# ktncktnc/diffusion-forcing-transformer

Hardware: AMD Instinct MI355X
Metric: denoised latent frames/sec, DFoT RE10K 8f & 200f rollout @1/2/4/8 GPU (higher is better)
Workload: dtype bf16

## Files before the change

diffusion-forcing-transformer_amd/backbone.py:

```python
from __future__ import annotations

import ctypes as C
import math
from typing import Dict, Optional, Sequence, Tuple

import torch
from torch import nn

from . import capi, ops


def _get(cfg, key, default=None):
    if isinstance(cfg, dict):
        return cfg.get(key, default)
    return getattr(cfg, key, default) if not hasattr(cfg, "get") else cfg.get(key, default)


class _Node(nn.Module):
    """Anonymous container so that dotted reference key names map onto a module tree."""


class UViT3DPose(nn.Module):
    def __init__(self, cfg, x_shape: Sequence[int], max_tokens: int, external_cond_dim: int = 0,
                 external_cond_type: str = "action", external_cond_num_classes: Optional[int] = None,
                 use_causal_mask: bool = False, **kwargs):
        super().__init__()
        block_types = list(_get(cfg, "block_types", ["ResBlock", "ResBlock", "TransformerBlock", "TransformerBlock"]))
        if block_types != ["ResBlock", "ResBlock", "TransformerBlock", "TransformerBlock"]:
            raise ValueError(f"unsupported block_types {block_types}")
        if _get(cfg, "pos_emb_type", "rope") != "rope":
            raise ValueError("only pos_emb_type='rope' is supported")
        if not _get(cfg, "use_fourier_noise_embedding", True):
            raise ValueError("only the Fourier noise-level embedding (continuous diffusion) is supported")
        cond = _get(cfg, "conditioning", None)
        cond_dim = _get(cond, "dim", None) if cond is not None else None
        self.cfg = cfg
        self.x_shape = tuple(x_shape)
        self.max_tokens = self.temporal_length = int(max_tokens)
        self.external_cond_dim = int(cond_dim or 180)
        self.use_causal_mask = use_causal_mask
        c = capi.UViTConfig()
        c.channels[:] = list(_get(cfg, "channels"))
        c.emb_channels = int(_get(cfg, "emb_channels"))
        c.num_updown_blocks[:] = list(_get(cfg, "num_updown_blocks"))
        c.num_mid_blocks = int(_get(cfg, "num_mid_blocks"))
        c.num_heads = int(_get(cfg, "num_heads"))
        c.in_channels = int(self.x_shape[0])
        c.resolution = int(self.x_shape[-1])
        c.max_tokens = self.max_tokens
        c.cond_dim = self.external_cond_dim
        c.noise_dim = 256
        c.rope_theta = 10000.0
        c.eps = 1e-6
        if int(_get(cfg, "patch_size", 2)) != 2:
            raise ValueError("only patch_size=2 is supported")
        self._ccfg = c
        self._handle = C.c_void_p()
        capi.check(capi.lib.dfot_uvit_create(C.byref(c), C.byref(self._handle)))
        self._names = []
        self._persistent_buffers = {"noise_level_pos_embedding.timesteps.freqs",
                                    "noise_level_pos_embedding.timesteps.phases"}
        shape = (C.c_int64 * 4)()
        ndim = C.c_int()
        for i in range(capi.lib.dfot_uvit_num_params(self._handle)):
            name = capi.lib.dfot_uvit_param_name(self._handle, i).decode()
            capi.check(capi.lib.dfot_uvit_param_shape(self._handle, i, shape, C.byref(ndim)))
            self._register(name, tuple(shape[k] for k in range(ndim.value)))
            self._names.append(name)
        self._synced: Optional[Tuple] = None
        self._reserved = 0
        self._op_key: Optional[int] = None
        self._cond_key = None
        self._cond_refs = None
        self._cond_gen = None
        self._cond_flag = None
        self.cond_cache_stats = {"builds": 0, "identity_hits": 0, "content_hits": 0}
        self._train_names = None
        self._trainer = None
        self._trainer_sig = None
        self.live_frames = None
        self.fresh_frames = None
        self._fresh_key = None
        self._train_stamp = 0
        self._dropout_generator: Optional[torch.Generator] = None

    def _register(self, name: str, shape: Tuple[int, ...]) -> None:
        *path, leaf = name.split(".")
        node: nn.Module = self
        for part in path:
            if part not in node._modules:
                node.add_module(part, _Node())
            node = node._modules[part]
        t = torch.zeros(shape, dtype=torch.float32)
        if name in self._persistent_buffers:
            node.register_buffer(leaf, t, persistent=True)
        else:
            node.register_parameter(leaf, nn.Parameter(t))

    def _tensors(self) -> Dict[str, torch.Tensor]:
        sd = dict(self.named_parameters())
        sd.update(dict(self.named_buffers()))
        return sd

    def reset_parameters(self, seed: int = 0) -> None:
        g = torch.Generator().manual_seed(seed)
        with torch.no_grad():
            for name, t in self._tensors().items():
                leaf = name.rsplit(".", 1)[-1]
                if leaf == "freqs":
                    t.copy_(2 * math.pi * torch.randn(t.shape, generator=g))
                elif leaf == "phases":
                    t.copy_(2 * math.pi * torch.rand(t.shape, generator=g))
                elif any(s in name for s in (".attn_out.", ".mlp_out.2.", ".out_rest.1.", "project_output")):
                    t.zero_()
                elif leaf == "bias":
                    t.zero_()
                elif t.ndim == 1:
                    t.fill_(1.0)
                else:
                    fan_in = math.prod(t.shape[1:])
                    bound = 1.0 / math.sqrt(fan_in)
                    t.copy_((torch.rand(t.shape, generator=g) * 2 - 1) * bound)

    def _signature(self) -> Tuple:
        return tuple((t.data_ptr(), t._version) for t in self._tensors().values())

    def sync_weights(self, force: bool = False) -> None:
        sig = self._signature()
        if not force and sig == self._synced:
            return
        tensors = self._tensors()
        s = capi.stream_ptr()
        for name in self._names:
            t = tensors[name]
            if not t.is_cuda:
                raise RuntimeError(f"parameter {name} is on {t.device}; move the module to the GPU first")
            src = t.detach().to(torch.float32).contiguous()
            shape = (C.c_int64 * src.ndim)(*src.shape)
            capi.check(capi.lib.dfot_uvit_load_weight(self._handle, name.encode(), capi.ptr(src), shape, src.ndim, s))
        capi.check(capi.lib.dfot_uvit_finalize(self._handle, s))
        self._synced = sig
        self.reserve_generation = getattr(self, "reserve_generation", 0) + 1

    def set_option(self, key: str, value: int) -> None:
        self.reserve_generation = getattr(self, "reserve_generation", 0) + 1
        capi.check(capi.lib.dfot_uvit_set_option(self._handle, key.encode(), int(value)))

    def query(self, key: str) -> float:
        self.sync_weights()
        val = C.c_double()
        capi.check(capi.lib.dfot_uvit_query(self._handle, key.encode(), C.byref(val)))
        return float(val.value)

    def attn_timing(self):
        tot, n = C.c_double(), C.c_int64()
        capi.check(capi.lib.dfot_uvit_attn_timing(self._handle, C.byref(tot), C.byref(n)))
        return tot.value, n.value

    def init_random(self, seed: int = 0, zero_init_scale: float = 0.3) -> None:
        g = torch.Generator().manual_seed(seed)
        with torch.no_grad():
            for name, t in self._tensors().items():
                leaf = name.rsplit(".", 1)[-1]
                if leaf == "freqs":
# ... 10 lines not shown
                    if any(s in name for s in (".attn_out.", ".mlp_out.2.", ".out_rest.1.", "project_output")):
                        v = v * zero_init_scale
                t.copy_(v.to(t.device))

    def reserve(self, batch: int) -> None:
        if batch > self._reserved:
            torch.cuda.synchronize()
            capi.check(capi.lib.dfot_uvit_reserve(self._handle, int(batch)))
            self._reserved = batch
            self.reserve_generation = getattr(self, "reserve_generation", 0) + 1
            self._cond_key = None

    def forward(self, x: torch.Tensor, noise_levels: torch.Tensor, external_cond: Optional[torch.Tensor] = None,
                external_cond_mask: Optional[torch.Tensor] = None) -> torch.Tensor:
        assert external_cond is not None, "External condition (camera pose) is required for U-ViT3DPose model."
        if self._op_key is None:
            self._op_key = ops.register_model(self)
        if torch.is_grad_enabled() and (x.requires_grad or any(p.requires_grad for p in self.parameters())):
            if self._train_names is None:
                self._train_names = [n for n, _ in self.named_parameters()]
            params = [p for _, p in self.named_parameters()]
            return torch.ops.dfot.uvit3d_pose_forward_train(x, noise_levels, external_cond, external_cond_mask, params, self._op_key)
        return torch.ops.dfot.uvit3d_pose_forward(x, noise_levels, external_cond, external_cond_mask, self._op_key)

    def _train_engine(self, params):
        from . import uvit_train
        sig = tuple((t.data_ptr(), t._version) for t in params) + tuple((b.data_ptr(), b._version) for _, b in self.named_buffers())
        if self._trainer is None:
            cfg = dict(channels=list(self._ccfg.channels), emb_channels=int(self._ccfg.emb_channels), patch_size=2,
                       block_types=["ResBlock", "ResBlock", "TransformerBlock", "TransformerBlock"],
                       num_updown_blocks=list(self._ccfg.num_updown_blocks), num_mid_blocks=int(self._ccfg.num_mid_blocks),
                       num_heads=int(self._ccfg.num_heads), in_channels=int(self._ccfg.in_channels), resolution=int(self._ccfg.resolution),
                       max_tokens=self.max_tokens, cond_dim=self.external_cond_dim, noise_dim=int(self._ccfg.noise_dim),
                       eps=float(self._ccfg.eps), rope_theta=float(self._ccfg.rope_theta),
                       block_dropouts=list(_get(self.cfg, "block_dropouts", [0.0] * 4) or [0.0] * 4))
            sd = {n: t for n, t in zip(self._train_names, params)}
            sd.update(dict(self.named_buffers()))
            ordered = {n: sd[n] for n in self._names}
            self._trainer = uvit_train.UViT3DPoseTrainer(ordered, cfg)
            self._trainer_sig = sig
        elif sig != self._trainer_sig:
            with torch.no_grad():
                for n, t in zip(self._train_names, params):
                    self._trainer.p[n].copy_(t)
                for n, b in self.named_buffers():
                    self._trainer.p[n].copy_(b)
            self._trainer.sync()
            self._trainer_sig = sig
        return self._trainer

    def _train_forward_impl(self, x, noise_levels, external_cond, external_cond_mask, params):
        assert x.shape[1] == self.temporal_length, (
            f"Temporal length of U-ViT is set to {self.temporal_length}, but input has temporal length {x.shape[1]}.")
        dev = params[0].device
        if dev.type != "cuda":
            raise RuntimeError(f"the backbone's parameters are on {dev}; move the module to the GPU first (there is no CPU path)")
        capi.require_device(dev, x=x, noise_levels=noise_levels, external_cond=external_cond, external_cond_mask=external_cond_mask)
        eng = self._train_engine(params)
        drop = external_cond_mask
        pdrop = float(_get(self.cfg, "external_cond_dropout", 0.0) or 0.0)
        if drop is None and self.training and pdrop > 0:
            drop = torch.rand(x.shape[0], device=dev) < pdrop
        eng.dropout_generator = self._dropout_generator if self.training else None
        self._train_stamp += 1
        with torch.no_grad():
            return eng.forward(x, noise_levels, external_cond, drop).to(x.dtype)

    def _train_backward_impl(self, grad_out, params, stamp=None, want_dx=False):
        eng = self._trainer
        if eng is None:
            raise RuntimeError("backward without a training forward")
        if stamp is not None and stamp != self._train_stamp:
            raise RuntimeError(
                f"UViT3DPose: backward of training forward #{stamp}, but forward #{self._train_stamp} has run since and overwritten the "
                "saved activations (one engine per module). Run backward after each forward (accumulate gradients as forward/backward "
                "pairs); two forwards of one module inside one loss are not supported.")
        with torch.no_grad():
            grads = eng.backward(grad_out, input_grad=want_dx)
        out = [grads[n].to(p.dtype).reshape(p.shape) if n in grads else torch.zeros_like(p) for n, p in zip(self._train_names, params)]
        if want_dx:
            out.append(eng.dx_in.to(grad_out.dtype))
        return out

    def _cond_content_equal(self, cond: torch.Tensor, mask: Optional[torch.Tensor]) -> bool:
        if self._cond_key is None or self._cond_refs is None:
            return False
        kept, kept_mask = self._cond_refs
        _, version, shape, synced, mask_key = self._cond_key
        if synced != self._synced or self._cond_gen != self.reserve_generation:
            return False
        if kept._version != version or (kept_mask is not None and kept_mask._version != mask_key[1]):
            return False
        for t in (cond, kept):
            if t.dtype != torch.float32 or not t.is_contiguous():
                return False
        if cond.device != kept.device or tuple(cond.shape) != shape:
            return False
        if (mask is None) != (kept_mask is None):
            return False
        if mask is not None and (mask.dtype != kept_mask.dtype or mask.shape != kept_mask.shape or mask.device != kept_mask.device
                                 or not mask.is_contiguous() or not kept_mask.is_contiguous()):
            return False
        if torch.cuda.is_current_stream_capturing():
            return False
        if self._cond_flag is None or self._cond_flag.device != cond.device:
            self._cond_flag = torch.zeros(1, dtype=torch.int32, device=cond.device)
        flag = self._cond_flag
        flag.zero_()
        s = capi.stream_ptr()
        capi.check(capi.lib.dfot_op_equal_bits(capi.ptr(kept), capi.ptr(cond), cond.numel() * cond.element_size(), capi.ptr(flag), s))
        if mask is not None:
            capi.check(capi.lib.dfot_op_equal_bits(capi.ptr(kept_mask), capi.ptr(mask), mask.numel() * mask.element_size(), capi.ptr(flag), s))
        return int(flag.item()) == 0

    def _forward_impl(self, x: torch.Tensor, noise_levels: torch.Tensor, external_cond: Optional[torch.Tensor] = None,
                      external_cond_mask: Optional[torch.Tensor] = None) -> torch.Tensor:
        assert x.shape[1] == self.temporal_length, (
            f"Temporal length of U-ViT is set to {self.temporal_length}, but input has temporal length {x.shape[1]}.")
        assert external_cond is not None, "External condition (camera pose) is required for U-ViT3DPose model."
        b = x.shape[0]
        if tuple(x.shape[2:]) != self.x_shape:
            raise ValueError(f"x has frame shape {tuple(x.shape[2:])}, expected {self.x_shape}")
        if tuple(external_cond.shape) != (b, self.temporal_length, self.external_cond_dim, *self.x_shape[1:]):
            raise ValueError(f"external_cond has shape {tuple(external_cond.shape)}")
        if external_cond_mask is not None:
            assert external_cond_mask.ndim == 1, "embedding mask should be of shape (B,)"
        if tuple(noise_levels.shape) != (b, self.temporal_length):
            raise ValueError(f"noise_levels has shape {tuple(noise_levels.shape)}, expected {(b, self.temporal_length)}")
        dev = next(self.parameters()).device
        if dev.type != "cuda":
            raise RuntimeError(f"the backbone's parameters are on {dev}; move the module to the GPU first (there is no CPU path)")
        capi.require_device(dev, x=x, noise_levels=noise_levels, external_cond=external_cond, external_cond_mask=external_cond_mask)
        self.sync_weights()
        self.reserve(b)
        xf = x.detach().to(torch.float32).contiguous()
        kf = noise_levels.detach().to(torch.float32).contiguous()
        key = (external_cond.data_ptr(), external_cond._version, tuple(external_cond.shape), self._synced,
               None if external_cond_mask is None else (external_cond_mask.data_ptr(), external_cond_mask._version))
        if key == self._cond_key:
            self.cond_cache_stats["identity_hits"] += 1
        else:
            if self._cond_content_equal(external_cond, external_cond_mask):
                self.cond_cache_stats["content_hits"] += 1
            else:
                cf = external_cond.detach().to(torch.float32).contiguous()
                mf = None if external_cond_mask is None else external_cond_mask.to(torch.uint8).contiguous()
                capi.check(capi.lib.dfot_uvit_set_conditions(self._handle, capi.ptr(cf, torch.float32, "external_cond"),
                                                             capi.ptr(mf, torch.uint8, "external_cond_mask"), b, capi.stream_ptr()))
                self.cond_cache_stats["builds"] += 1
            self._cond_key = key
            self._cond_refs = (external_cond, external_cond_mask)
            self._cond_gen = self.reserve_generation
        out = torch.empty_like(xf)
        live = self.live_frames
        if live is not None:
            if tuple(live.shape) != (b, self.temporal_length) or live.dtype != torch.uint8 or not live.is_contiguous():
                raise ValueError(f"live_frames must be a contiguous uint8 tensor of shape {(b, self.temporal_length)}")
            capi.require_device(dev, live_frames=live)
        fresh = self.fresh_frames
        if fresh is not None:
            if tuple(fresh.shape) != (b, self.temporal_length) or fresh.dtype != torch.uint8 or not fresh.is_contiguous():
                raise ValueError(f"fresh_frames must be a contiguous uint8 tensor of shape {(b, self.temporal_length)}")
            capi.require_device(dev, fresh_frames=fresh)
            if key != self._fresh_key:
                fresh = None
        capi.check(capi.lib.dfot_uvit_forward_cached_masks(self._handle, capi.ptr(xf, torch.float32, "x"),
                                                           capi.ptr(kf, torch.float32, "noise_levels"), capi.ptr(out), b,
                                                           capi.ptr(live, torch.uint8, "live_frames"),
                                                           capi.ptr(fresh, torch.uint8, "fresh_frames"), capi.stream_ptr()))
        self._fresh_key = key
        return out.to(x.dtype)

    def read_tap(self, name: str, channels: int, level: int, batch: int) -> torch.Tensor:
        r = self.x_shape[-1] // 2 // (2 ** level)
        out = torch.empty(batch * self.temporal_length, channels, r, r, device="cuda", dtype=torch.float32)
        capi.check(capi.lib.dfot_uvit_read_tap(self._handle, name.encode(), capi.ptr(out), out.numel(), capi.stream_ptr()))
        return out

    def __del__(self):
        try:
            if getattr(self, "_handle", None) and self._handle.value:
                capi.lib.dfot_uvit_destroy(self._handle)
                self._handle = C.c_void_p()
        except Exception:
            pass
```

diffusion-forcing-transformer_amd/capi.py:

```python
from __future__ import annotations

import ctypes as C
import os

_HERE = os.path.dirname(os.path.abspath(__file__))
LIB_PATH = os.environ.get("DFOT_LIB", os.path.join(_HERE, "libdfot_hip.so"))

OK, ERR_ARG, ERR_SHAPE, ERR_HIP, ERR_STATE, ERR_NAME = range(6)


class DfotError(RuntimeError):
    def __init__(self, code: int, message: str):
        super().__init__(f"libdfot_hip error {code}: {message}")
        self.code = code


class UViTConfig(C.Structure):
    _fields_ = [
        ("channels", C.c_int32 * 4), ("emb_channels", C.c_int32), ("num_updown_blocks", C.c_int32 * 3),
        ("num_mid_blocks", C.c_int32), ("num_heads", C.c_int32), ("in_channels", C.c_int32),
        ("resolution", C.c_int32), ("max_tokens", C.c_int32), ("cond_dim", C.c_int32), ("noise_dim", C.c_int32),
        ("rope_theta", C.c_float), ("eps", C.c_float),
    ]


class UViT3DConfig(C.Structure):
    _fields_ = UViTConfig._fields_ + [("cond_dropout", C.c_int32)]


class DiTConfig(C.Structure):
    _fields_ = [
        ("hidden_size", C.c_int32), ("depth", C.c_int32), ("num_heads", C.c_int32), ("patch_size", C.c_int32),
        ("in_channels", C.c_int32), ("height", C.c_int32), ("width", C.c_int32), ("max_tokens", C.c_int32),
        ("mlp_hidden", C.c_int32), ("noise_dim", C.c_int32), ("timesteps", C.c_int32),
        ("rope_theta", C.c_float), ("eps", C.c_float),
        ("variant", C.c_int32), ("embed_col_dim", C.c_int32), ("num_col_heads", C.c_int32), ("num_row_heads", C.c_int32),
        ("temporal_mlp_hidden", C.c_int32), ("use_bias", C.c_int32),
        ("cond_type", C.c_int32), ("cond_dim", C.c_int32), ("num_classes", C.c_int32), ("cond_dropout", C.c_int32),
        ("use_temporal_rope", C.c_int32),
    ]


class DiTConfigF(DiTConfig):
    _fields_ = [("fourier_noise", C.c_int32)]


COND_NONE, COND_ACTION, COND_LABEL = 0, 1, 2
ATTN_MAP_OFF, ATTN_MAP_FRAME, ATTN_MAP_FULL = -1, 0, 1


_P, _I, _L, _F = C.c_void_p, C.c_int, C.c_int64, C.c_float
_I32 = C.c_int32


class GemmDesc(C.Structure):
    _fields_ = [
        ("amode", _I32), ("epi", _I32), ("variant", _I32),
        ("A", _P), ("lda", _L), ("W", _P), ("ldw", _L),
        ("M", _I32), ("N", _I32), ("K", _I32), ("H", _I32), ("Wd", _I32), ("Cin", _I32),
        ("live", _P), ("bias", _P), ("bias_rows", _I32),
        ("out_f32", _P), ("out_bf16", _P), ("ldo", _L),
        ("resid", _P), ("resid_bf", _P),
        ("gate", _P), ("gate_index", _P), ("ldg", _L), ("gate_rows", _I32),
        ("act", _I32), ("pre_act", _P), ("raw", _P), ("ldraw", _L), ("tr_rows", _I32),
        ("gn_part", _P), ("gn_rows_per_bt", _I32), ("gn_cpg", _I32),
        ("out2", _P), ("ldo2", _L), ("split", _I32),
        ("q", _P), ("k", _P), ("v", _P),
        ("qw", _P), ("kw", _P), ("rope_cs", _P),
        ("heads", _I32), ("d", _I32), ("ntok", _I32), ("qscale", _F), ("dstride", _I32), ("eps", _F),
        ("ksplit", _I32), ("slice_stride", _L),
    ]


SIGNATURES = {
    "dfot_last_error": (C.c_char_p, []),
    "dfot_version": (_I, []),
    "dfot_uvit_create": (_I, [C.POINTER(UViTConfig), C.POINTER(_P)]),
    "dfot_uvit_destroy": (_I, [_P]),
    "dfot_uvit_num_params": (_I, [_P]),
    "dfot_uvit_param_name": (C.c_char_p, [_P, _I]),
    "dfot_uvit_param_shape": (_I, [_P, _I, C.POINTER(_L), C.POINTER(_I)]),
    "dfot_uvit_load_weight": (_I, [_P, C.c_char_p, _P, C.POINTER(_L), _I, _P]),
    "dfot_uvit_finalize": (_I, [_P, _P]),
    "dfot_uvit_reserve": (_I, [_P, _I]),
    "dfot_uvit_workspace_bytes": (C.c_size_t, [_P]),
    "dfot_uvit_set_option": (_I, [_P, C.c_char_p, _I]),
    "dfot_uvit_query": (_I, [_P, C.c_char_p, C.POINTER(C.c_double)]),
    "dfot_uvit_attn_timing": (_I, [_P, C.POINTER(C.c_double), C.POINTER(_L)]),
    "dfot_uvit_forward": (_I, [_P, _P, _P, _P, _P, _P, _I, _P]),
    "dfot_uvit_set_conditions": (_I, [_P, _P, _P, _I, _P]),
    "dfot_uvit_forward_cached": (_I, [_P, _P, _P, _P, _I, _P]),
    "dfot_uvit_forward_cached_live": (_I, [_P, _P, _P, _P, _I, _P, _P]),
    "dfot_uvit_forward_cached_masks": (_I, [_P, _P, _P, _P, _I, _P, _P, _P]),
    "dfot_uvit_read_tap": (_I, [_P, C.c_char_p, _P, C.c_size_t, _P]),
    "dfot_uvit3d_create": (_I, [C.POINTER(UViT3DConfig), C.POINTER(_P)]),
    "dfot_uvit3d_config_bytes": (_L, []),
    "dfot_uvit3d_forward": (_I, [_P, _P, _P, _P, _P, _P, _I, _P]),
    "dfot_uvit3d_forward_live": (_I, [_P, _P, _P, _P, _P, _P, _I, _P, _P]),
    "dfot_op_gn_film_silu": (_I, [_P, _P, _P, _P, _P, _P, _P, _P, _I, _I, _I, _I, _P]),
    "dfot_op_rms_film": (_I, [_P, _P, _P, _P, _P, _P, _L, _I, _I, _I, _F, _P]),
    "dfot_dit_create": (_I, [C.POINTER(DiTConfig), C.POINTER(_P)]),
    "dfot_dit_create_f": (_I, [C.POINTER(DiTConfigF), C.POINTER(_P)]),
    "dfot_dit_destroy": (_I, [_P]),
    "dfot_dit_num_params": (_I, [_P]),
    "dfot_dit_param_name": (C.c_char_p, [_P, _I]),
    "dfot_dit_param_shape": (_I, [_P, _I, C.POINTER(_L), C.POINTER(_I)]),
    "dfot_dit_load_weight": (_I, [_P, C.c_char_p, _P, C.POINTER(_L), _I, _P]),
    "dfot_dit_finalize": (_I, [_P, _P]),
    "dfot_dit_reserve": (_I, [_P, _I]),
    "dfot_dit_workspace_bytes": (C.c_size_t, [_P]),
    "dfot_dit_set_option": (_I, [_P, C.c_char_p, _I]),
    "dfot_dit_attn_timing": (_I, [_P, C.POINTER(C.c_double), C.POINTER(_L)]),
    "dfot_dit_forward": (_I, [_P, _P, _P, _P, _I, _I, _P]),
    "dfot_dit_forward_cond": (_I, [_P, _P, _P, _P, _P, _P, _P, _I, _I, _P]),
    "dfot_dit_forward_f": (_I, [_P, _P, _P, _P, _P, _P, _P, _I, _I, _P]),
    "dfot_dit_read_tap": (_I, [_P, C.c_char_p, _P, C.c_size_t, _P]),
    "dfot_dit_capture_attention": (_I, [_P, C.POINTER(_I32), _I, _I, C.c_size_t]),
    "dfot_dit_attention_map_shape": (_I, [_P, _I, C.POINTER(_L), C.POINTER(_I)]),
    "dfot_dit_read_attention_map": (_I, [_P, _I, _P, C.c_size_t, _P]),
    "dfot_dit_train_create": (_I, [C.POINTER(DiTConfig), C.POINTER(_P)]),
    "dfot_dit_train_create_f": (_I, [C.POINTER(DiTConfigF), C.POINTER(_P)]),
    "dfot_facmat_train_create": (_I, [C.POINTER(DiTConfigF), C.POINTER(_P)]),
    "dfot_facdit_train_create": (_I, [C.POINTER(DiTConfigF), C.POINTER(_P)]),
    "dfot_dit_train_destroy": (_I, [_P]),
    "dfot_dit_train_num_params": (_I, [_P]),
    "dfot_dit_train_param_name": (C.c_char_p, [_P, _I]),
    "dfot_dit_train_param_shape": (_I, [_P, _I, C.POINTER(_L), C.POINTER(_I)]),
    "dfot_dit_train_param_offset": (_L, [_P, _I]),
    "dfot_dit_train_total_numel": (_L, [_P]),
    "dfot_dit_train_workspace_bytes": (C.c_size_t, [_P]),
    "dfot_dit_train_attach": (_I, [_P, _P, _P]),
    "dfot_dit_train_reserve": (_I, [_P, _I]),
    "dfot_dit_train_sync_weights": (_I, [_P, _P]),
    "dfot_dit_train_forward": (_I, [_P, _P, _P, _P, _I, _I, _P]),
    "dfot_dit_train_forward_cond": (_I, [_P, _P, _P, _P, _P, _P, _P, _I, _I, _P]),
    "dfot_dit_train_load_buffer": (_I, [_P, C.c_char_p, _P, _L, _P]),
    "dfot_dit_train_forward_f": (_I, [_P, _P, _P, _P, _P, _P, _P, _I, _I, _P]),
    "dfot_dit_train_input_grad": (_I, [_P, _P, _P]),
    "dfot_dit_train_backward": (_I, [_P, _P, _P]),
    "dfot_vloss_grad": (_I, [_P] * 7 + [_I, _I, _L, _I, _P]),
    "dfot_sumsq": (_I, [_P, _L, _P, _P]),
    "dfot_adamw_step": (_I, [_P, _P, _P, _P, _L, _F, _F, _F, _F, _F, _I, _P, _F, _P, _F, _P]),
    "dfot_ray_encode": (_I, [_P, _P, _I, _I, _I, _P]),
    "dfot_ray_encode_normalized": (_I, [_P, _P, _I, _I, _I, _P]),
    "dfot_hg_prepare": (_I, [_P, _P, _P, _P, _P, _I, _I, _I, _L, _P]),
    "dfot_ddim_compose": (_I, [_P] * 11 + [_I, _I, _I, _L, _P]),
    "dfot_ddim_compose_tokw": (_I, [_P] * 11 + [_I, _I, _I, _L, _P]),
    "dfot_ddim_noise": (_I, [_P] * 5 + [_I, _I, _I, _L, _I, _P]),
    "dfot_vpred_loss": (_I, [_P] * 9 + [_I, _I, _L, _P]),
    "dfot_vpred_loss_scratch_floats": (_L, [_I, _I, _L]),
    "dfot_vspace_loss": (_I, [_P] * 9 + [_I, _I, _L, _P]),
    "dfot_op_gemm": (_I, [_P, _I, _P, _P, _P, _I, _I, _I, _I, _P]),
    "dfot_op_conv3x3": (_I, [_P, _P, _P, _P, _I, _I, _I, _I, _I, _I, _P]),
    "dfot_op_gemm_ex": (_I, [C.POINTER(GemmDesc), _P]),
    "dfot_op_gemm_desc_bytes": (_L, []),
    "dfot_op_attention": (_I, [_P, _P, _P, _P, _I, _I, _I, _I, _I, _I, _P]),
    "dfot_op_attention_padded": (_I, [_P, _P, _P, _P, _I, _I, _I, _I, _I, _P]),
    "dfot_op_attention_seq64": (_I, [_P, _P, _P, _P, _I, _I, _I, _I, _P]),
    "dfot_op_attention_temporal": (_I, [_P, _P, _P, _P, _I, _I, _I, _I, _I, _I, _P]),
    "dfot_op_attention_temporal_bwd": (_I, [_P, _P, _P, _P, _I, _P, _P, _P, _I, _I, _I, _I, _I, _P]),
    "dfot_op_matrix_attention_rope": (_I, [_P, _P, _P, _I, _I, _I, _I, _I, _I, _F, _P]),
    "dfot_op_matrix_attention_rope_bwd": (_I, [_P, _P, _P, _P, _I, _I, _I, _I, _I, _I, _F, _P]),
    "dfot_op_attention_map_workspace_bytes": (C.c_size_t, [_I, _I, _I, _I, _I]),
    "dfot_op_attention_map": (_I, [_P, _P, _P, _P, C.c_size_t, _I, _I, _I, _I, _I, _I, _P]),
    "dfot_op_attention_temporal_map": (_I, [_P, _P, _P, _P, C.c_size_t, _I, _I, _I, _I, _I, _P]),
    "dfot_op_matrix_attention_map": (_I, [_P, _P, _P, _I, _I, _I, _I, _I, _I, _F, _P]),
    "dfot_op_matrix_attention": (_I, [_P, _P, _I, _I, _I, _I, _I, _I, _F, _P]),
    "dfot_op_facmat_contract": (_I, [_P, _P, _P, _I, _I, _I, _I, _P]),
    "dfot_op_facmat_expand": (_I, [_P, _P, _P, _I, _I, _I, _I, _P]),
    "dfot_op_attention_bwd": (_I, [_P, _P, _P, _P, _P, _I, _P, _P, _P, _I, _I, _I, _I, _P]),
    "dfot_op_conv3x3_bwd": (_I, [_P, _P, _P, _P, _P, _P, _I, _I, _I, _I, _I, _P]),
    "dfot_op_conv3x3_bwd2": (_I, [_P, _P, _P, _P, _P, _P, _P, _I, _I, _I, _I, _I, _P]),
    "dfot_op_gn_silu_bwd": (_I, [_P, _P, _P, _P, _P, _F, _P, _P, _P, _P, _I, _I, _I, _P]),
    "dfot_op_rms_film_bwd": (_I, [_P, _P, _P, _P, _F, _P, _P, _P, _L, _I, _I, _P]),
    "dfot_op_rms_film_bwd_res": (_I, [_P, _P, _P, _P, _F, _P, _P, _P, _P, _P, _L, _I, _P]),
    "dfot_op_qknorm_rope_bwd": (_I, [_P, _I, _P, _P, _P, _P, _P, _P, _F, _P, _I, _P, _P, _L, _I, _I, _I, _P]),
    "dfot_op_wgrad_nt": (_I, [_P, _I, _P, _I, _P, _I, _I, _L, _I, _P]),
    "dfot_op_gemm_bf16": (_I, [_P, _I, _P, _P, _P, _I, _I, _I, _I, _P]),
    "dfot_op_gemm_f32": (_I, [_P, _I, _P, _P, _P, _P, _I, _I, _I, _I, _P]),
    "dfot_op_transpose_bf16": (_I, [_P, _P, _I, _I, _P]),
    "dfot_op_colsum_bf16": (_I, [_P, _I, _P, _L, _I, _P]),
    "dfot_op_rms_film_fwd": (_I, [_P, _P, _P, _F, _P, _L, _I, _P]),
    "dfot_op_qknorm_rope_fwd": (_I, [_P, _I, _P, _P, _P, _F, _F, _P, _P, _P, _L, _I, _I, _I, _P]),
# ... 116 lines not shown
```

diffusion-forcing-transformer_amd/csrc/kernels.h:

```cpp
#pragma once
#include "common.h"

namespace dfot {

int launch_noise_emb(const float* k, const float* freqs, const float* phases, const float* w1, const float* b1,
                     const float* w2, const float* b2, float* hidden, float* out, int bt, int ndim, int e, hipStream_t s);
int launch_uvit3d_emb(const float* k, const float* freqs, const float* phases, const float* w1, const float* b1, const float* w2,
                      const float* b2, const float* cond, const uint8_t* cond_mask, const float* a_w1, const float* a_b1,
                      const float* a_w2, const float* a_b2, float* out, int bt, int ndim, int cdim, int e, int tokens, hipStream_t s);
int launch_embed_input(const float* x, const float* w, const float* b, float* out, int bt, int res, int cin, int c0,
                       hipStream_t s);
int launch_cond_repack(const float* cond, bf16* a, int bt, int res, int cdim, int kpad, hipStream_t s);
int launch_emb_pyramid(const bf16* emb0, bf16* emb1, bf16* emb2, bf16* emb3, int bt, int r0, int e, hipStream_t s);
int launch_project_output(const float* x0, const float* w, const float* b, float* out, int bt, int res, int c0, int cout,
                          hipStream_t s, const uint8_t* live = nullptr);
int launch_gn_partial_f32(const float* x, float* partial, int bt, int pixels, int c, hipStream_t s);
int launch_gn_partial_bf16(const bf16* x, float* partial, int bt, int pixels, int c, hipStream_t s);
int launch_gn_finalize(const float* partial, float* stats, int bt, int nblk, int pixels, int c, float eps, hipStream_t s);
int gn_partial_blocks(int pixels);
int launch_gn_apply_silu(const float* x, const float* stats, const float* gamma, const float* beta, bf16* out, int bt,
                         int pixels, int c, hipStream_t s, const uint8_t* live = nullptr);
struct FilmChunk {
  const bf16* w;
  const float* b;
  long out_off;
  int rows;
};
int launch_film_vec(const FilmChunk* table, int chunks, const float* nemb, float* sv, int bt, int e, hipStream_t s);
int launch_gn_film_silu(const bf16* h, const float* stats, const float* gamma, const float* beta, const bf16* fcache,
                        const float* sv, const uint8_t* cond_mask, bf16* out, int bt, int pixels, int c, int tokens,
                        hipStream_t s, const uint8_t* live = nullptr);
struct RmsPending {
  void* x;
  const float* bias;
  const float* s0;
  const float* s1;
  const float* s2;
};
int launch_rms_film(const float* x, const float* w, const bf16* fcache, const float* sv, const uint8_t* cond_mask, bf16* out,
                    long m, int c, int rows_per_bt, int tokens, float eps, hipStream_t s, const RmsPending* pend = nullptr);
int launch_rms_film_bf16(const bf16* x, const float* w, const bf16* fcache, const float* sv, const uint8_t* cond_mask, bf16* out,
                         long m, int c, int rows_per_bt, int tokens, float eps, hipStream_t s, const RmsPending* pend = nullptr);

int launch_pool2_bf16(const float* x, bf16* out, int bt, int h, int w, int c, hipStream_t s);
int launch_pool2_bf16_bf16in(const bf16* x, bf16* out, int bt, int h, int w, int c, hipStream_t s);
int launch_sub_bf16_bf16in(const bf16* a, const float* b, bf16* out, long n, hipStream_t s, const uint8_t* live = nullptr, long frame_elems = 0);
int launch_upsample_add_bf16(const float* t, const bf16* skip, bf16* out, int bt, int h, int w, int c, hipStream_t s, const uint8_t* live = nullptr);
int launch_gn_apply_silu_bf16in(const bf16* x, const float* stats, const float* gamma, const float* beta, bf16* out, int bt, int pixels, int c,
                                hipStream_t s, const uint8_t* live = nullptr);
int launch_embed_input_bf16(const float* x, const float* w, const float* b, bf16* out, int bt, int res, int cin, int c0, hipStream_t s);
int launch_project_output_bf16(const bf16* x0, const float* w, const float* b, float* out, int bt, int res, int c0, int cout, hipStream_t s,
                               const uint8_t* live = nullptr);
int launch_sub_bf16(const float* a, const float* b, bf16* out, long n, hipStream_t s, const uint8_t* live = nullptr, long frame_elems = 0);
int launch_upsample_add(const float* t, const float* skip, float* out, int bt, int h, int w, int c, hipStream_t s, const uint8_t* live = nullptr);
int launch_ray_encode(const float* poses, float* out, int b, int t, int res, int normalized, hipStream_t s);
int launch_hg_prepare(const float* x, const float* noise, const float* qa, const float* qb, float* x_in, int batch,
                      int nfe, int tokens, long f, hipStream_t s);
int launch_ddim_compose(const float* x, const float* x_in, const float* v, const float* sa, const float* s1,
                        const float* an, const float* cn, const float* keep, const float* weight, const uint8_t* gen,
                        float* x_next, int batch, int nfe, int tokens, long f, bool weight_per_token, hipStream_t s);
int launch_ddim_noise(const float* noise, const float* sigma, const float* weight, const uint8_t* gen, float* x_next, int batch, int nfe,
                      int tokens, long f, bool weight_per_token, hipStream_t s);
int vloss_chunks(long f);
int launch_vloss(const float* x, const float* noise, const float* v, const float* a, const float* sg, const float* w,
                 float* x_pred, float* partial, float* loss, int batch, int tokens, long f, bool vspace, hipStream_t s);
int launch_wgrad_nt(const bf16* a, long lda, const bf16* b, long ldb, float* out, int m, int n, long rows, int slices, hipStream_t s, int img_h = 0,
                    int img_w = 0, int sdy = 0, int sdx = 0, int all_taps = 0);
struct WgradPlan {
  int form, slices;
};
WgradPlan wgrad_plan(int m, int n, long rows, long max_slices);
int launch_wgrad_conv_taps(const bf16* dy, const bf16* x, float* out, int co, int ci, long pix, int slices, int img_h, int img_w, hipStream_t s);
int wgrad_conv_tiles(int co, int ci, int* target);
int launch_wgrad_nt_plan(const bf16* a, long lda, const bf16* b, long ldb, float* out, int m, int n, long rows, WgradPlan plan, hipStream_t s);
int launch_vloss_grad(const float* x, const float* noise, const float* v, const float* a, const float* sg, const float* coef, float* dv,
                      int batch, int tokens, long f, bool vspace, hipStream_t s);
int launch_sumsq(const float* x, long n, float* out, hipStream_t s);
int launch_adamw(float* p, const float* g, float* m, float* v, long n, float lr, float b1, float b2, float eps, float wd, int step,
                 const float* sumsq, float max_norm, float* ema, float ema_decay, hipStream_t s);
int launch_f32_to_bf16(const float* src, bf16* dst, long n, hipStream_t s);
int launch_bf16_to_f32(const bf16* src, float* dst, long n, hipStream_t s);
int launch_equal_bits(const void* a, const void* b, long bytes, int* differs, hipStream_t s);
int launch_pack_rows(const float* src, bf16* dst, const int* map, int rows, int k, int kpad, long ldd, int col0,
                     hipStream_t s);
int launch_pack_conv3(const float* src, bf16* dst, int co, int ci, hipStream_t s);
int launch_gather_f32(const float* src, float* dst, const int* map, int n, hipStream_t s);
int launch_nhwc_to_nchw(const float* src, float* dst, int bt, int p, int c, hipStream_t s);
int launch_bf16_nhwc_to_nchw(const bf16* src, float* dst, int bt, int p, int c, hipStream_t s);

struct AttnScratch {
  float* p = nullptr;
  size_t bytes = 0;
};
int launch_attention(const bf16* q, const bf16* k, const bf16* v, bf16* o, long ldo, int batch, int heads, int n, int d,
                     int variant, hipStream_t stream, AttnScratch* scratch = nullptr);
int launch_attention_v3(const bf16* q, const bf16* k, const bf16* v, bf16* o, long ldo, int batch, int heads, int n, bool nomax,
                        hipStream_t stream, AttnScratch* scratch = nullptr);
bool attention_v5_applies(int n, int d, float score_bound);
int launch_attention_v5(const bf16* q, const bf16* k, const bf16* v, bf16* o, long ldo, int batch, int heads, int n, hipStream_t stream,
                        AttnScratch* scratch = nullptr, float* lse = nullptr);
bool attention_ks_applies(int batch, int heads, int n, int d);
size_t attention_ks_scratch_bytes(int batch, int heads, int n, int d);
int launch_attention_ks(const bf16* q, const bf16* k, const bf16* v, bf16* o, long ldo, int batch, int heads, int n, hipStream_t stream,
                        AttnScratch* scratch = nullptr);
int attention_dstride(int d);
int launch_attention_padded(const bf16* q, const bf16* k, const bf16* v, bf16* o, long ldo, int batch, int heads, int n, int d,
                            hipStream_t stream, float* lse = nullptr);
int launch_attention_seq64(const bf16* q, const bf16* k, const bf16* v, bf16* o, long ldo, int nseq, int heads, int d, hipStream_t stream);
int launch_attention_temporal(const bf16* q, const bf16* k, const bf16* v, bf16* o, long ldo, int batch, int tokens, int patches, int heads,
                              int d, hipStream_t s);
int launch_attention_temporal_bwd(const bf16* q, const bf16* k, const bf16* v, const bf16* d_o, long ldo, bf16* dq, bf16* dk, bf16* dv,
                                  int batch, int tokens, int patches, int heads, int d, hipStream_t s);
int launch_matrix_attn_rope(const bf16* z, bf16* o, const float* rope_cs, int batch, int L, int E, int h, int cc, int rr, float scale,
                            hipStream_t s);
int launch_matrix_attn_rope_bwd(const bf16* z, const bf16* d_o, const float* rope_cs, bf16* dz, int batch, int L, int E, int h, int cc, int rr,
                                float scale, hipStream_t s);
int launch_facmat_contract(const bf16* m, const bf16* u, bf16* w, int frames, int P, int h, int E, hipStream_t s);
int launch_facmat_expand(const bf16* o, const bf16* u, bf16* sp, int frames, int P, int h, int E, hipStream_t s);
size_t attention_map_part_floats(int batch, int heads, int n, int tokens);
int launch_attention_map(const bf16* q, const bf16* k, float* out, float* part, bool full, int batch, int heads, int n, int tokens, int d,
                         hipStream_t s);
size_t attention_temporal_map_part_floats(int batch, int heads, int tokens, int patches);
int launch_attention_temporal_map(const bf16* q, const bf16* k, float* out, float* part, int batch, int tokens, int patches, int heads, int d,
                                  hipStream_t s);
int launch_matrix_attn_map(const bf16* z, const float* rope_cs, float* out, int batch, int L, int E, int h, int cc, int rr, float scale,
// ... 17 lines not shown
```

diffusion-forcing-transformer_amd/csrc/kernels.hip:

```cpp
#include "kernels.h"
#include "dfot_hip.h"

namespace dfot {

typedef __attribute__((ext_vector_type(4))) float float4v;
typedef __attribute__((ext_vector_type(2))) float float2v;

__device__ __forceinline__ float wave_sum(float v) {
#pragma unroll
  for (int o = 32; o > 0; o >>= 1) v += __shfl_xor(v, o);
  return v;
}

template <bool FOURIER>
__global__ __launch_bounds__(256) void noise_mlp_kernel(const float* __restrict__ in, const float* __restrict__ freqs,
                                                        const float* __restrict__ phases, const float* __restrict__ w,
                                                        const float* __restrict__ b, float* __restrict__ out, int kdim,
                                                        int e) {
  const int lane = threadIdx.x & 63, wave = threadIdx.x >> 6;
  const int row = blockIdx.x * 4 + wave;
  const int bt = blockIdx.y;
  if (row >= e) return;
  float acc = 0.f;
  for (int i = lane; i < kdim; i += 64) {
// ... 638 lines not shown
    const float* ne = nemb + (long)bt * e;
    float acc = 0.f;
#pragma unroll
    for (int k = 0; k < 2; ++k) {
      const int i = lane * 8 + k * 512;
      if (i < e) {
        const float4v a = *reinterpret_cast<const float4v*>(ne + i);
        const float4v b = *reinterpret_cast<const float4v*>(ne + i + 4);
        acc += wv[k][0] * a[0] + wv[k][1] * a[1] + wv[k][2] * a[2] + wv[k][3] * a[3] + wv[k][4] * b[0] + wv[k][5] * b[1] +
               wv[k][6] * b[2] + wv[k][7] * b[3];
      }
    }
    acc = wave_sum(acc);
    if (lane == 0) sv[ck.out_off + (long)bt * ck.rows + r] = acc + bias;
  }
}
template <int EQ>
__global__ __launch_bounds__(256, 2) void film_vec_lds_kernel(const FilmChunk* __restrict__ table, const float* __restrict__ nemb,
                                                           float* __restrict__ sv, int nbt) {
  constexpr int E = EQ * 256;
  __shared__ float4v ne[16][E / 4];
  const FilmChunk ck = table[blockIdx.x >> 1];
  const int lane = threadIdx.x & 63, wave = threadIdx.x >> 6;
  for (int bt0 = 0; bt0 < nbt; bt0 += 16) {
    __syncthreads();
    for (int i = threadIdx.x; i < 16 * (E / 4); i += 256) {
      const int f = i / (E / 4);
      float4v v = {0.f, 0.f, 0.f, 0.f};
      if (bt0 + f < nbt) v = reinterpret_cast<const float4v*>(nemb + (long)(bt0 + f) * E)[i % (E / 4)];
      ne[f][i % (E / 4)] = v;
    }
    __syncthreads();
#pragma unroll 1
    for (int pass = 0; pass < 4; ++pass) {
      const int r0 = (blockIdx.x & 1) * 32 + pass * 8 + wave * 2;
      float wv[2][EQ][4];
#pragma unroll
      for (int r = 0; r < 2; ++r)
#pragma unroll
        for (int k = 0; k < EQ; ++k) {
          const bf16x4 t = *reinterpret_cast<const bf16x4*>(ck.w + (long)(r0 + r) * E + k * 256 + lane * 4);
#pragma unroll
          for (int j = 0; j < 4; ++j) wv[r][k][j] = bf2f(t[j]);
        }
      float acc[32];
#pragma unroll
      for (int f = 0; f < 16; ++f) {
        float4v x[EQ];
#pragma unroll
        for (int k = 0; k < EQ; ++k) x[k] = ne[f][k * 64 + lane];
#pragma unroll
        for (int r = 0; r < 2; ++r) {
          float a = 0.f;
#pragma unroll
          for (int k = 0; k < EQ; ++k) a += wv[r][k][0] * x[k][0] + wv[r][k][1] * x[k][1] + wv[r][k][2] * x[k][2] + wv[r][k][3] * x[k][3];
          acc[r * 16 + f] = a;
        }
        if ((f & 3) == 3) __builtin_amdgcn_sched_barrier(0);
      }
      halve_exchange<16, 32>(acc, lane);
      halve_exchange<8, 16>(acc, lane);
      halve_exchange<4, 8>(acc, lane);
      halve_exchange<2, 4>(acc, lane);
      halve_exchange<1, 2>(acc, lane);
      const float v = acc[0] + __shfl_xor(acc[0], 1);
      const int r = r0 + (lane >> 5), f = bt0 + ((lane >> 1) & 15);
      if (f < nbt && (lane & 1) == 0) sv[ck.out_off + (long)f * ck.rows + r] = v + ck.b[r];
    }
  }
}
int launch_film_vec(const FilmChunk* table, int chunks, const float* nemb, float* sv, int bt, int e, hipStream_t s) {
  DFOT_REQUIRE(e % 8 == 0 && e <= 1024, DFOT_ERR_SHAPE, "film_vec: emb dim %d must be a multiple of 8 and <= 1024", e);
  if (e == 1024 || e == 512) {
    if (e == 1024) hipLaunchKernelGGL(film_vec_lds_kernel<4>, dim3(chunks * 2), dim3(256), 0, s, table, nemb, sv, bt);
    else hipLaunchKernelGGL(film_vec_lds_kernel<2>, dim3(chunks * 2), dim3(256), 0, s, table, nemb, sv, bt);
    DFOT_CHECK_HIP(hipGetLastError());
    return DFOT_OK;
  }
  hipLaunchKernelGGL(film_vec_kernel, dim3(chunks * 16), dim3(256), 0, s, table, nemb, sv, e, bt);
  DFOT_CHECK_HIP(hipGetLastError());
  return DFOT_OK;
}

template <bool POSE>
__global__ void gn_film_silu_kernel(const bf16* __restrict__ h, const float* __restrict__ stats,
                                    const float* __restrict__ gamma, const float* __restrict__ beta,
                                    const bf16* __restrict__ fcache, const float* __restrict__ sv,
                                    const uint8_t* __restrict__ cond_mask, bf16* __restrict__ out, long total8, int pixels,
                                    int c, int tokens, const uint8_t* __restrict__ live) {
  const long idx = (long)blockIdx.x * blockDim.x + threadIdx.x;
  if (idx >= total8) return;
  const unsigned iu = (unsigned)idx, cq = (unsigned)(c / 8);
  const int c8 = (int)(iu % cq);
  const long pix = iu / cq;
  const int bt = (int)((unsigned)pix / (unsigned)pixels);
  if (live && !live[bt]) return;
  const int cpg = c / 32;
  const int c0 = c8 * 8;
  const int col = (c0 >> 5) * 64 + (c0 & 31);
  const bf16x8 hv = *reinterpret_cast<const bf16x8*>(h + pix * c + c0);
  const float* svp = sv + (long)bt * 2 * c + col;
  float sc[8], sh[8];
#pragma unroll
  for (int j = 0; j < 8; ++j) {
    sc[j] = svp[j];
    sh[j] = svp[32 + j];
  }
  if constexpr (POSE) {
    const bool use_pose = !(cond_mask && cond_mask[(unsigned)bt / (unsigned)tokens]);
    if (use_pose) {
      const bf16x8 fs = *reinterpret_cast<const bf16x8*>(fcache + pix * 2 * c + col);
      const bf16x8 fh = *reinterpret_cast<const bf16x8*>(fcache + pix * 2 * c + col + 32);
#pragma unroll
      for (int j = 0; j < 8; ++j) {
        sc[j] += bf2f(fs[j]);
        sh[j] += bf2f(fh[j]);
      }
    }
  }
  bf16x8 o;
#pragma unroll
  for (int j = 0; j < 8; ++j) {
    const int ch = c0 + j;
    const int g = ch / cpg;
    const float mean = stats[(bt * 32 + g) * 2], rs = stats[(bt * 32 + g) * 2 + 1];
    const float y = ((bf2f(hv[j]) - mean) * rs * gamma[ch] + beta[ch]) * (1.f + sc[j]) + sh[j];
    o[j] = f2bf(silu_f(y));
  }
  *reinterpret_cast<bf16x8*>(out + pix * c + c0) = o;
}
template <int C, bool POSE>
__global__ __launch_bounds__(256) void gn_film_silu_rows_kernel(const bf16* __restrict__ h, const float* __restrict__ stats,
                                                                const float* __restrict__ gamma, const float* __restrict__ beta,
                                                                const bf16* __restrict__ fcache, const float* __restrict__ sv,
                                                                const uint8_t* __restrict__ cond_mask, bf16* __restrict__ out, int pixels,
                                                                int tokens, const uint8_t* __restrict__ live) {
  constexpr int TPP = C / 8, PPI = 256 / TPP;
  const int wg_per_bt = pixels / (PPI * GN_ROWS_IT);
  const int bt = blockIdx.x / wg_per_bt;
  if (live && !live[bt]) return;
  const int c0 = (threadIdx.x % TPP) * 8;
  const int col = (c0 >> 5) * 64 + (c0 & 31);
  GnRowConsts<C> k;
  k.load(stats, gamma, beta, bt, c0);
  const float* svp = sv + (long)bt * 2 * C + col;
  float svs[8], svh[8];
  {
    const float4v s0 = *reinterpret_cast<const float4v*>(svp), s1 = *reinterpret_cast<const float4v*>(svp + 4);
    const float4v h0 = *reinterpret_cast<const float4v*>(svp + 32), h1 = *reinterpret_cast<const float4v*>(svp + 36);
#pragma unroll
    for (int j = 0; j < 8; ++j) {
      svs[j] = j < 4 ? s0[j] : s1[j - 4];
      svh[j] = j < 4 ? h0[j] : h1[j - 4];
    }
  }
  bool use_pose = false;
  if constexpr (POSE) use_pose = !(cond_mask && cond_mask[(unsigned)bt / (unsigned)tokens]);
  long pix = (long)bt * pixels + (long)(blockIdx.x % wg_per_bt) * (PPI * GN_ROWS_IT) + threadIdx.x / TPP;
  if (POSE && use_pose) {
#pragma unroll 4
    for (int it = 0; it < GN_ROWS_IT; ++it, pix += PPI) {
      const bf16x8 hv = *reinterpret_cast<const bf16x8*>(h + pix * C + c0);
      const bf16x8 fs = *reinterpret_cast<const bf16x8*>(fcache + pix * 2 * C + col);
      const bf16x8 fh = *reinterpret_cast<const bf16x8*>(fcache + pix * 2 * C + col + 32);
      bf16x8 o;
#pragma unroll
      for (int j = 0; j < 8; ++j) {
        const float sc = svs[j] + bf2f(fs[j]), sh = svh[j] + bf2f(fh[j]);
        o[j] = f2bf(silu_f(k.norm(bf2f(hv[j]), j) * (1.f + sc) + sh));
      }
      *reinterpret_cast<bf16x8*>(out + pix * C + c0) = o;
    }
  } else {
#pragma unroll 4
    for (int it = 0; it < GN_ROWS_IT; ++it, pix += PPI) {
      const bf16x8 hv = *reinterpret_cast<const bf16x8*>(h + pix * C + c0);
      bf16x8 o;
#pragma unroll
      for (int j = 0; j < 8; ++j) o[j] = f2bf(silu_f(k.norm(bf2f(hv[j]), j) * (1.f + svs[j]) + svh[j]));
      *reinterpret_cast<bf16x8*>(out + pix * C + c0) = o;
    }
  }
}

template <bool POSE>
static int launch_gn_film_silu_t(const bf16* h, const float* stats, const float* gamma, const float* beta, const bf16* fcache,
                                 const float* sv, const uint8_t* cond_mask, bf16* out, int bt, int pixels, int c, int tokens,
                                 hipStream_t s, const uint8_t* live) {
  if ((c == 128 || c == 256) && pixels % ((256 / (c / 8)) * GN_ROWS_IT) == 0) {
    const int grid = bt * (pixels / ((256 / (c / 8)) * GN_ROWS_IT));
    if (c == 128)
      hipLaunchKernelGGL((gn_film_silu_rows_kernel<128, POSE>), dim3(grid), dim3(256), 0, s, h, stats, gamma, beta, fcache, sv, cond_mask, out, pixels, tokens, live);
    else
      hipLaunchKernelGGL((gn_film_silu_rows_kernel<256, POSE>), dim3(grid), dim3(256), 0, s, h, stats, gamma, beta, fcache, sv, cond_mask, out, pixels, tokens, live);
    DFOT_CHECK_HIP(hipGetLastError());
    return DFOT_OK;
  }
  const long total8 = (long)bt * pixels * (c / 8);
  DFOT_REQUIRE(total8 < (1L << 31), DFOT_ERR_SHAPE, "groupnorm apply: %ld work items exceed the 32-bit index range", total8);
  hipLaunchKernelGGL(gn_film_silu_kernel<POSE>, dim3(cdiv(total8, 256)), dim3(256), 0, s, h, stats, gamma, beta, fcache, sv,
                     cond_mask, out, total8, pixels, c, tokens, live);
  DFOT_CHECK_HIP(hipGetLastError());
  return DFOT_OK;
}
int launch_gn_film_silu(const bf16* h, const float* stats, const float* gamma, const float* beta, const bf16* fcache,
                        const float* sv, const uint8_t* cond_mask, bf16* out, int bt, int pixels, int c, int tokens,
                        hipStream_t s, const uint8_t* live) {
  return fcache ? launch_gn_film_silu_t<true>(h, stats, gamma, beta, fcache, sv, cond_mask, out, bt, pixels, c, tokens, s, live)
                : launch_gn_film_silu_t<false>(h, stats, gamma, beta, nullptr, sv, nullptr, out, bt, pixels, c, tokens, s, live);
}

template <int MAXCH, bool PEND, typename TS, bool POSE>
__global__ __launch_bounds__(256) void rms_film_kernel(const TS* x, const float* __restrict__ w,
                                                       const bf16* __restrict__ fcache, const float* __restrict__ sv,
                                                       const uint8_t* __restrict__ cond_mask, bf16* __restrict__ out,
                                                       long m, int c, int rows_per_bt, int tokens, float eps, TS* xw,
                                                       const float* __restrict__ pbias, const float* __restrict__ p0,
                                                       const float* __restrict__ p1, const float* __restrict__ p2) {
  const long row = (long)blockIdx.x * 4 + (threadIdx.x >> 6);
  if (row >= m) return;
  const int lane = threadIdx.x & 63;
  const int nch = c / 8;
  const TS* src = x + row * c;
  float v[MAXCH][8];
  float ss = 0.f;
#pragma unroll
  for (int k = 0; k < MAXCH; ++k) {
    const int ch = lane + 64 * k;
    if (ch < nch) {
      stream_ld8(src + ch * 8, v[k]);
      if constexpr (PEND) {
        const long o = row * c + ch * 8;
#pragma unroll
        for (int hf = 0; hf < 2; ++hf) {
          float4v add = *reinterpret_cast<const float4v*>(pbias + ch * 8 + 4 * hf) + *reinterpret_cast<const float4v*>(p0 + o + 4 * hf) +
                        *reinterpret_cast<const float4v*>(p1 + o + 4 * hf);
          if (p2) add += *reinterpret_cast<const float4v*>(p2 + o + 4 * hf);
#pragma unroll
          for (int j = 0; j < 4; ++j) v[k][4 * hf + j] += add[j];
        }
        stream_st8(xw + o, v[k]);
        if constexpr (sizeof(TS) == 2) {
#pragma unroll
          for (int j = 0; j < 8; ++j) v[k][j] = bf2f(f2bf(v[k][j]));
        }
      }
#pragma unroll
      for (int j = 0; j < 8; ++j) ss += v[k][j] * v[k][j];
    }
  }
  ss = wave_sum(ss);
  const float rs = rsqrtf(ss / (float)c + eps);
  const int bt = (int)(row / rows_per_bt);
  bool use_pose = false;
  if constexpr (POSE) use_pose = !(cond_mask && cond_mask[(unsigned)bt / (unsigned)tokens]);
#pragma unroll
  for (int k = 0; k < MAXCH; ++k) {
    const int ch = lane + 64 * k;
    if (ch < nch) {
      const int c0 = ch * 8;
      const int col = (c0 >> 5) * 64 + (c0 & 31);
      const float* svp = sv + (long)bt * 2 * c + col;
      float sc[8], sh[8];
#pragma unroll
      for (int j = 0; j < 8; ++j) {
        sc[j] = svp[j];
        sh[j] = svp[32 + j];
      }
      if (POSE && use_pose) {
        const bf16x8 fs = *reinterpret_cast<const bf16x8*>(fcache + row * 2 * c + col);
        const bf16x8 fh = *reinterpret_cast<const bf16x8*>(fcache + row * 2 * c + col + 32);
#pragma unroll
        for (int j = 0; j < 8; ++j) {
          sc[j] += bf2f(fs[j]);
          sh[j] += bf2f(fh[j]);
        }
      }
      bf16x8 o;
#pragma unroll
      for (int j = 0; j < 8; ++j) o[j] = f2bf(v[k][j] * rs * w[c0 + j] * (1.f + sc[j]) + sh[j]);
      *reinterpret_cast<bf16x8*>(out + row * c + c0) = o;
    }
  }
}
template <typename TS, bool POSE>
static int launch_rms_film_p(const TS* x, const float* w, const bf16* fcache, const float* sv, const uint8_t* cond_mask, bf16* out,
                             long m, int c, int rows_per_bt, int tokens, float eps, hipStream_t s, const RmsPending* pend) {
  DFOT_REQUIRE(c % 8 == 0 && c <= 8 * 64 * 3, DFOT_ERR_SHAPE, "rms_film: channels %d unsupported", c);
#define RMS_CALL(MC, P)                                                                                                             \
  hipLaunchKernelGGL((rms_film_kernel<MC, P, TS, POSE>), dim3(cdiv(m, 4)), dim3(256), 0, s, x, w, fcache, sv, cond_mask, out, m, c, rows_per_bt, \
                     tokens, eps, P ? (TS*)pend->x : nullptr, P ? pend->bias : nullptr, P ? pend->s0 : nullptr, P ? pend->s1 : nullptr, P ? pend->s2 : nullptr)
  if (pend) {
    DFOT_REQUIRE(pend->x && pend->bias && pend->s0 && pend->s1, DFOT_ERR_ARG, "rms_film: pending sum needs a target, a bias and two slices");
    if (c <= 8 * 64 * 2) RMS_CALL(2, true); else RMS_CALL(3, true);
  } else {
    if (c <= 8 * 64 * 2) RMS_CALL(2, false); else RMS_CALL(3, false);
  }
#undef RMS_CALL
  DFOT_CHECK_HIP(hipGetLastError());
  return DFOT_OK;
}
template <typename TS>
static int launch_rms_film_t(const TS* x, const float* w, const bf16* fcache, const float* sv, const uint8_t* cond_mask, bf16* out,
                             long m, int c, int rows_per_bt, int tokens, float eps, hipStream_t s, const RmsPending* pend) {
  return fcache ? launch_rms_film_p<TS, true>(x, w, fcache, sv, cond_mask, out, m, c, rows_per_bt, tokens, eps, s, pend)
                : launch_rms_film_p<TS, false>(x, w, nullptr, sv, nullptr, out, m, c, rows_per_bt, tokens, eps, s, pend);
}
int launch_rms_film(const float* x, const float* w, const bf16* fcache, const float* sv, const uint8_t* cond_mask, bf16* out,
                    long m, int c, int rows_per_bt, int tokens, float eps, hipStream_t s, const RmsPending* pend) {
  return launch_rms_film_t<float>(x, w, fcache, sv, cond_mask, out, m, c, rows_per_bt, tokens, eps, s, pend);
}
int launch_rms_film_bf16(const bf16* x, const float* w, const bf16* fcache, const float* sv, const uint8_t* cond_mask, bf16* out,
                         long m, int c, int rows_per_bt, int tokens, float eps, hipStream_t s, const RmsPending* pend) {
  return launch_rms_film_t<bf16>(x, w, fcache, sv, cond_mask, out, m, c, rows_per_bt, tokens, eps, s, pend);
}

template <typename TIN>
__global__ void pool2_bf16_kernel(const TIN* __restrict__ x, bf16* __restrict__ out, long total4, int h, int w, int c) {
  const long idx = (long)blockIdx.x * blockDim.x + threadIdx.x;
  if (idx >= total4) return;
  const unsigned iu = (unsigned)idx, cq = (unsigned)(c / 4), w2 = (unsigned)(w / 2), h2 = (unsigned)(h / 2);
  const int c4 = (int)(iu % cq);
  const unsigned pix = iu / cq;
  const int ox = (int)(pix % w2), oy = (int)((pix / w2) % h2);
  const long bt = pix / (w2 * h2);
  const TIN* base = x + ((bt * h + 2 * oy) * w + 2 * ox) * (long)c + c4 * 4;
  const float4v a = stream_ld4(base);
  const float4v b = stream_ld4(base + c);
  const float4v cc = stream_ld4(base + (long)w * c);
  const float4v dd = stream_ld4(base + (long)w * c + c);
  bf16x4 o;
#pragma unroll
  for (int j = 0; j < 4; ++j) o[j] = f2bf((a[j] + b[j] + cc[j] + dd[j]) * 0.25f);
  *reinterpret_cast<bf16x4*>(out + pix * c + c4 * 4) = o;
}
int launch_pool2_bf16(const float* x, bf16* out, int bt, int h, int w, int c, hipStream_t s) {
  const long total4 = (long)bt * (h / 2) * (w / 2) * (c / 4);
  DFOT_REQUIRE(total4 < (1L << 31), DFOT_ERR_SHAPE, "pool2: %ld work items exceed the 32-bit index range", total4);
  hipLaunchKernelGGL(pool2_bf16_kernel<float>, dim3(cdiv(total4, 256)), dim3(256), 0, s, x, out, total4, h, w, c);
  DFOT_CHECK_HIP(hipGetLastError());
  return DFOT_OK;
}
int launch_pool2_bf16_bf16in(const bf16* x, bf16* out, int bt, int h, int w, int c, hipStream_t s) {
  const long total4 = (long)bt * (h / 2) * (w / 2) * (c / 4);
  DFOT_REQUIRE(total4 < (1L << 31), DFOT_ERR_SHAPE, "pool2: %ld work items exceed the 32-bit index range", total4);
  hipLaunchKernelGGL(pool2_bf16_kernel<bf16>, dim3(cdiv(total4, 256)), dim3(256), 0, s, x, out, total4, h, w, c);
  DFOT_CHECK_HIP(hipGetLastError());
  return DFOT_OK;
}

template <typename TIN, typename TB = TIN>
__global__ void sub_bf16_kernel(const TIN* __restrict__ a, const TB* __restrict__ b, bf16* __restrict__ out, long n4,
                                const uint8_t* __restrict__ live, long frame4) {
  const long idx = (long)blockIdx.x * blockDim.x + threadIdx.x;
  if (idx >= n4) return;
  if (live && !live[idx / frame4]) return;
  const float4v x = stream_ld4(a + idx * 4);
  const float4v y = stream_ld4(b + idx * 4);
  bf16x4 o;
#pragma unroll
  for (int j = 0; j < 4; ++j) o[j] = f2bf(x[j] - y[j]);
  *reinterpret_cast<bf16x4*>(out + idx * 4) = o;
}
int launch_sub_bf16(const float* a, const float* b, bf16* out, long n, hipStream_t s, const uint8_t* live, long frame_elems) {
  DFOT_REQUIRE(n % 4 == 0 && (!live || (frame_elems > 0 && frame_elems % 4 == 0)), DFOT_ERR_SHAPE, "sub: length %ld must be a multiple of 4", n);
  hipLaunchKernelGGL((sub_bf16_kernel<float, float>), dim3(cdiv(n / 4, 256)), dim3(256), 0, s, a, b, out, n / 4, live, live ? frame_elems / 4 : 1L);
  DFOT_CHECK_HIP(hipGetLastError());
  return DFOT_OK;
}
int launch_sub_bf16_bf16in(const bf16* a, const float* b, bf16* out, long n, hipStream_t s, const uint8_t* live, long frame_elems) {
  DFOT_REQUIRE(n % 4 == 0 && (!live || (frame_elems > 0 && frame_elems % 4 == 0)), DFOT_ERR_SHAPE, "sub: length %ld must be a multiple of 4", n);
  hipLaunchKernelGGL((sub_bf16_kernel<bf16, float>), dim3(cdiv(n / 4, 256)), dim3(256), 0, s, a, b, out, n / 4, live, live ? frame_elems / 4 : 1L);
  DFOT_CHECK_HIP(hipGetLastError());
  return DFOT_OK;
}

template <typename TS>
__global__ void upsample_add_kernel(const float* __restrict__ t, const TS* __restrict__ skip, TS* __restrict__ out,
                                    long total4, int h, int w, int c, const uint8_t* __restrict__ live) {
  const long idx = (long)blockIdx.x * blockDim.x + threadIdx.x;
  if (idx >= total4) return;
  const unsigned iu = (unsigned)idx, cq = (unsigned)(c / 4), w2 = (unsigned)(2 * w), h2 = (unsigned)(2 * h);
  const int c4 = (int)(iu % cq);
  const unsigned pix = iu / cq;
  const int x = (int)(pix % w2), y = (int)((pix / w2) % h2);
  const long bt = pix / (w2 * h2);
  if (live && !live[bt]) return;
  const float4v a = *reinterpret_cast<const float4v*>(t + ((bt * h + y / 2) * w + x / 2) * (long)c + c4 * 4);
  const float4v b = stream_ld4(skip + pix * c + c4 * 4);
  stream_st4(out + pix * c + c4 * 4, a + b);
}
int launch_upsample_add(const float* t, const float* skip, float* out, int bt, int h, int w, int c, hipStream_t s, const uint8_t* live) {
  const long total4 = (long)bt * 4 * h * w * (c / 4);
  DFOT_REQUIRE(total4 < (1L << 31), DFOT_ERR_SHAPE, "upsample_add: %ld work items exceed the 32-bit index range", total4);
  hipLaunchKernelGGL(upsample_add_kernel<float>, dim3(cdiv(total4, 256)), dim3(256), 0, s, t, skip, out, total4, h, w, c, live);
  DFOT_CHECK_HIP(hipGetLastError());
  return DFOT_OK;
// ... 495 lines not shown
```

diffusion-forcing-transformer_amd/csrc/uvit.hip:

```cpp
#include <algorithm>
#include <cmath>
#include <cstdarg>
#include <cstdlib>
#include <cstring>
#include <functional>
#include <map>
#include <string>
#include <vector>

#include "dfot_hip.h"
#include "gemm.h"
#include "kernels.h"

namespace dfot {

static thread_local char g_err[1024] = "";
void set_error(const char* fmt, ...) {
  va_list ap;
  va_start(ap, fmt);
  vsnprintf(g_err, sizeof(g_err), fmt, ap);
  va_end(ap);
}
const char* get_error() { return g_err; }

int tuning_flag(const char* name, int dflt) {
  std::string key = std::string("DFOT_") + name;
  const char* v = getenv(key.c_str());
  return v ? atoi(v) : dflt;
}

struct ResW {
  int c = 0;
  bf16* fcache = nullptr;
  long sv_off = 0;
  bf16 *w_film = nullptr, *w1 = nullptr, *w2 = nullptr;
  float *b_film_raw = nullptr, *b_film = nullptr, *g1 = nullptr, *be1 = nullptr, *bias1 = nullptr, *g2 = nullptr,
        *be2 = nullptr, *bias2 = nullptr;
};
struct TrW {
  int c = 0;
  bf16* fcache = nullptr;
  long sv_off = 0;
  bf16 *w_film = nullptr, *w_fused = nullptr, *w_out = nullptr;
  float *b_film_raw = nullptr, *b_film = nullptr, *nw = nullptr, *b_fused = nullptr, *qw = nullptr, *kw = nullptr,
        *b_attn = nullptr, *b_mlp = nullptr, *b_out = nullptr;
  float score_bound = INFINITY;
};
struct ConvW {
  int cin = 0, cout = 0;
  bf16* w = nullptr;
  float* b = nullptr;
};

struct Param {
  std::string name;
  std::vector<int64_t> shape;
  std::function<int(const float*, hipStream_t)> load;
  bool loaded = false;
};

}

using namespace dfot;

struct dfot_uvit_s {
  dfot_uvit_config cfg{};
  int T = 0, E = 0, heads = 0, r[4] = {0, 0, 0, 0}, ch[4] = {0, 0, 0, 0};
  int kpose = 0;
  bool posefree = false;
  int act_dim = 0;
  bool act_dropout = false;
  float *ac_w1 = nullptr, *ac_b1 = nullptr, *ac_w2 = nullptr, *ac_b2 = nullptr;
  std::vector<Param> params;
  std::map<std::string, int> index;
  std::vector<void*> owned;

  float *ne_freqs = nullptr, *ne_phases = nullptr, *ne_w1 = nullptr, *ne_b1 = nullptr, *ne_w2 = nullptr, *ne_b2 = nullptr;
  bf16* pose_w = nullptr;
  float* pose_b = nullptr;
  float *ein_w = nullptr, *ein_b = nullptr, *pout_w = nullptr, *pout_b = nullptr;
  std::vector<ResW> down_res[2], up_res[2];
  std::vector<TrW> down_tr, mid_tr, up_tr;
  ConvW down_conv[3], up_conv[3];
  int* film_map[4] = {nullptr, nullptr, nullptr, nullptr};
  float* rope_cs[4] = {nullptr, nullptr, nullptr, nullptr};
  bf16* zeros = nullptr;
  bool finalized = false;

  int max_batch = 0;
  size_t ws_bytes = 0;
  std::vector<void*> ws_owned;
  float *nemb = nullptr, *nhid = nullptr, *X[4] = {nullptr, nullptr, nullptr, nullptr}, *HSA[3] = {nullptr, nullptr, nullptr}, *tmp = nullptr,
        *gn_partial = nullptr, *gn_partial2 = nullptr, *gn_stats = nullptr, *sv = nullptr;
  int gn1_nblk = 0;
  FilmChunk* film_table = nullptr;
  int film_chunks = 0;
  uint8_t* cond_mask = nullptr;
  bool have_mask = false;
  int cond_batch = 0;
  int64_t cond_builds = 0;
  bf16 *acond = nullptr, *emb[4] = {nullptr, nullptr, nullptr, nullptr}, *s1 = nullptr, *hbf = nullptr,
       *cat = nullptr, *q = nullptr, *k = nullptr, *v = nullptr;
  AttnScratch attn_scratch;
  const float* pend_part = nullptr;
  float* out_part = nullptr;
  size_t out_part_elems = 0;
  const float* pend_bias = nullptr;
  int pend_lvl = 0, pend_c = 0, pend_slices = 2;
  long pend_m = 0;
  int last_batch = 0;
  const float* xin[4] = {nullptr, nullptr, nullptr, nullptr};
  bf16* XB[4] = {nullptr, nullptr, nullptr, nullptr};
  bool xin_bf[4] = {false, false, false, false};
  int gemm_variant = GEMM_AUTO;
  int attn_variant = 2;
  bool attn_force_safe = false;
  bool time_attn = false;
  std::vector<hipEvent_t> ev_start, ev_stop;
  size_t ev_used = 0;
};

namespace dfot {

template <typename T>
static int dev_alloc(dfot_uvit_s* h, T** out, size_t count, bool workspace = false) {
  void* p = nullptr;
  const size_t bytes = count * sizeof(T);
  DFOT_CHECK_HIP(hipMalloc(&p, bytes ? bytes : 16));
  (workspace ? h->ws_owned : h->owned).push_back(p);
  if (workspace) h->ws_bytes += bytes;
  *out = reinterpret_cast<T*>(p);
  return DFOT_OK;
}

static int copy_f32(float* dst, const float* src, size_t n, hipStream_t s) {
  DFOT_CHECK_HIP(hipMemcpyAsync(dst, src, n * sizeof(float), hipMemcpyDeviceToDevice, s));
  return DFOT_OK;
}

static void add_param(dfot_uvit_s* h, const std::string& name, std::vector<int64_t> shape,
                      std::function<int(const float*, hipStream_t)> load) {
  h->index[name] = (int)h->params.size();
  h->params.push_back(Param{name, std::move(shape), std::move(load), false});
}

static int add_f32(dfot_uvit_s* h, const std::string& name, std::vector<int64_t> shape, float** dst) {
  size_t n = 1;
  for (auto d : shape) n *= (size_t)d;
  int rc = dev_alloc(h, dst, n);
  if (rc) return rc;
  float* d = *dst;
  add_param(h, name, shape, [d, n](const float* src, hipStream_t s) { return copy_f32(d, src, n, s); });
  return DFOT_OK;
}

static int add_res_block(dfot_uvit_s* h, const std::string& pre, int c, ResW* w) {
  const int e = h->E;
  w->c = c;
  int rc = 0;
  if ((rc = dev_alloc(h, &w->w_film, (size_t)2 * c * e))) return rc;
  if ((rc = dev_alloc(h, &w->b_film_raw, (size_t)2 * c))) return rc;
  if ((rc = dev_alloc(h, &w->b_film, (size_t)2 * c))) return rc;
  if ((rc = dev_alloc(h, &w->w1, (size_t)c * 9 * c))) return rc;
  if ((rc = dev_alloc(h, &w->w2, (size_t)c * 9 * c))) return rc;
  const int lvl = c == h->ch[0] ? 0 : 1;
  int* map = h->film_map[lvl];
  bf16* wf = w->w_film;
  add_param(h, pre + ".emb_layer.weight", {2 * c, e, 1, 1}, [=](const float* src, hipStream_t s) {
    return launch_pack_rows(src, wf, map, 2 * c, e, e, e, 0, s);
  });
  float *braw = w->b_film_raw, *bre = w->b_film;
  add_param(h, pre + ".emb_layer.bias", {2 * c}, [=](const float* src, hipStream_t s) {
    int r2 = copy_f32(braw, src, 2 * c, s);
    return r2 ? r2 : launch_gather_f32(braw, bre, map, 2 * c, s);
  });
  if ((rc = add_f32(h, pre + ".in_layers.0.weight", {c}, &w->g1))) return rc;
  if ((rc = add_f32(h, pre + ".in_layers.0.bias", {c}, &w->be1))) return rc;
  bf16* w1 = w->w1;
  add_param(h, pre + ".in_layers.2.weight", {c, c, 3, 3}, [=](const float* src, hipStream_t s) { return launch_pack_conv3(src, w1, c, c, s); });
  if ((rc = add_f32(h, pre + ".in_layers.2.bias", {c}, &w->bias1))) return rc;
  if ((rc = add_f32(h, pre + ".out_norm.weight", {c}, &w->g2))) return rc;
  if ((rc = add_f32(h, pre + ".out_norm.bias", {c}, &w->be2))) return rc;
// ... 122 lines not shown
  }
  auto add_mid = [&]() -> int {
    h->mid_tr.resize(c.num_mid_blocks);
    for (int i = 0; i < c.num_mid_blocks; ++i)
      if ((rc = add_tr_block(h, "mid_blocks." + std::to_string(i), 3, &h->mid_tr[i]))) return rc;
    return DFOT_OK;
  };
  if (!h->posefree && (rc = add_mid())) return rc;
  for (int j = 0; j < 3; ++j) {
    const int l = 2 - j;
    const int n = c.num_updown_blocks[l];
    const std::string pre = "up_blocks." + std::to_string(j) + ".";
    if ((rc = add_conv(h, pre + "0.conv", h->ch[l + 1], h->ch[l], &h->up_conv[l]))) return rc;
    if (l < 2) {
      h->up_res[l].resize(n);
      for (int i = 0; i < n; ++i)
        if ((rc = add_res_block(h, pre + std::to_string(i + 1), h->ch[l], &h->up_res[l][i]))) return rc;
    } else {
      h->up_tr.resize(n);
      for (int i = 0; i < n; ++i)
        if ((rc = add_tr_block(h, pre + std::to_string(i + 1), l, &h->up_tr[i]))) return rc;
    }
  }
  if (h->posefree && (rc = add_mid())) return rc;
  return DFOT_OK;
}

static int build_rope(dfot_uvit_s* h, int lvl) {
  const int d = h->ch[lvl] / h->heads, half = d / 2;
  const int q = half / 3, rem = half % 3;
  int parts[3] = {q, q, q};
  if (rem == 1) parts[0] = q + 1;
  if (rem == 2) parts[1] = parts[2] = q + 1;
  const int rr = h->r[lvl], n = h->T * rr * rr;
  std::vector<float> cs((size_t)n * half * 2);
  for (int tok = 0; tok < n; ++tok) {
    const int pos[3] = {tok / (rr * rr), (tok / rr) % rr, tok % rr};
    int pair = 0;
    for (int ax = 0; ax < 3; ++ax) {
      const int dim = 2 * parts[ax];
      for (int j = 0; j < parts[ax]; ++j, ++pair) {
        const float inv = 1.0f / powf(h->cfg.rope_theta, (float)(2 * j) / (float)dim);
        const float ang = (float)pos[ax] * inv;
        cs[((size_t)tok * half + pair) * 2 + 0] = cosf(ang);
        cs[((size_t)tok * half + pair) * 2 + 1] = sinf(ang);
      }
    }
  }
  int rc = dev_alloc(h, &h->rope_cs[lvl], cs.size());
  if (rc) return rc;
  DFOT_CHECK_HIP(hipMemcpy(h->rope_cs[lvl], cs.data(), cs.size() * sizeof(float), hipMemcpyHostToDevice));
  return DFOT_OK;
}

__global__ void add_vec_kernel(const float* a, const float* b, float* o, int n) {
  const int i = blockIdx.x * blockDim.x + threadIdx.x;
  if (i < n) o[i] = a[i] + b[i];
}

static int run_res_block(dfot_uvit_s* h, const ResW& w, int lvl, int bt, hipStream_t s, const uint8_t* live = nullptr) {
  const int c = w.c, rr = h->r[lvl], pix = rr * rr;
  const int m = bt * pix;
  const int slots = pix / 64;
  bf16* xb = h->XB[lvl];
  int rc = 0;
  if (!h->xin_bf[lvl]) {
    if ((rc = launch_f32_to_bf16(h->xin[lvl], xb, (long)m * c, s))) return rc;
    h->xin_bf[lvl] = true;
  }
  if (h->gn1_nblk == 0) {
    if ((rc = launch_gn_partial_bf16(xb, h->gn_partial, bt, pix, c, s))) return rc;
    h->gn1_nblk = gn_partial_blocks(pix);
  }
  if ((rc = launch_gn_finalize(h->gn_partial, h->gn_stats, bt, h->gn1_nblk, pix, c, h->cfg.eps, s))) return rc;
  h->gn1_nblk = 0;
  if ((rc = launch_gn_apply_silu_bf16in(xb, h->gn_stats, w.g1, w.be1, h->s1, bt, pix, c, s, live))) return rc;
  GemmArgs g;
  g.A = h->s1; g.W = w.w1; g.M = m; g.N = c; g.K = 9 * c; g.H = rr; g.Wd = rr; g.Cin = c; g.zeros = h->zeros;
  g.bias = w.bias1; g.out_bf16 = h->hbf; g.ldo = c; g.live = live;
  g.gn_part = h->gn_partial2; g.gn_rows_per_bt = pix; g.gn_cpg = c / 32;
  if ((rc = launch_gemm(A_CONV3, E_BF16, h->gemm_variant, g, s))) return rc;
  if ((rc = launch_gn_finalize(h->gn_partial2, h->gn_stats, bt, slots, pix, c, h->cfg.eps, s))) return rc;
  if ((rc = launch_gn_film_silu(h->hbf, h->gn_stats, w.g2, w.be2, w.fcache, h->sv + w.sv_off,
                                h->have_mask ? h->cond_mask : nullptr, h->s1, bt, pix, c, h->T, s, live)))
    return rc;
  GemmArgs o;
  o.A = h->s1; o.W = w.w2; o.M = m; o.N = c; o.K = 9 * c; o.H = rr; o.Wd = rr; o.Cin = c; o.zeros = h->zeros;
  o.bias = w.bias2; o.out_bf16 = xb; o.ldo = c; o.live = live;
  o.resid_bf = xb;
  o.gn_part = h->gn_partial; o.gn_rows_per_bt = pix; o.gn_cpg = c / 32;
  if ((rc = launch_gemm(A_CONV3, E_BF16, h->gemm_variant, o, s))) return rc;
  h->xin_bf[lvl] = true;
  h->gn1_nblk = slots;
  return DFOT_OK;
}

__global__ void out_reduce_kernel(bf16* x, const float* __restrict__ bias, const float* __restrict__ s0, const float* __restrict__ s1,
                                  const float* __restrict__ s2, long total4, int cq) {
  typedef __attribute__((ext_vector_type(4))) float f4;
  const long i = (long)blockIdx.x * blockDim.x + threadIdx.x;
  if (i >= total4) return;
  f4 b = reinterpret_cast<const f4*>(bias)[i % cq] + reinterpret_cast<const f4*>(s0)[i] + reinterpret_cast<const f4*>(s1)[i];
  if (s2) b += reinterpret_cast<const f4*>(s2)[i];
  const bf16x4 xv = reinterpret_cast<const bf16x4*>(x)[i];
  reinterpret_cast<bf16x4*>(x)[i] = bf16x4{f2bf(bf2f(xv[0]) + b[0]), f2bf(bf2f(xv[1]) + b[1]), f2bf(bf2f(xv[2]) + b[2]), f2bf(bf2f(xv[3]) + b[3])};
}
__global__ void add_f32_into_bf16_kernel(bf16* x, const float* __restrict__ y, long total4) {
  typedef __attribute__((ext_vector_type(4))) float f4;
  const long i = (long)blockIdx.x * blockDim.x + threadIdx.x;
  if (i >= total4) return;
  const f4 b = reinterpret_cast<const f4*>(y)[i];
  const bf16x4 xv = reinterpret_cast<const bf16x4*>(x)[i];
  reinterpret_cast<bf16x4*>(x)[i] = bf16x4{f2bf(bf2f(xv[0]) + b[0]), f2bf(bf2f(xv[1]) + b[1]), f2bf(bf2f(xv[2]) + b[2]), f2bf(bf2f(xv[3]) + b[3])};
}

static void swap_out_part(dfot_uvit_s* h) { h->pend_part = h->out_part; }

static int flush_pending(dfot_uvit_s* h, hipStream_t s) {
  if (!h->pend_bias) return DFOT_OK;
  const long total4 = h->pend_m * h->pend_c / 4;
  hipLaunchKernelGGL(out_reduce_kernel, dim3(cdiv(total4, 256)), dim3(256), 0, s, h->XB[h->pend_lvl], h->pend_bias, h->pend_part,
                     h->pend_part + h->pend_m * h->pend_c, h->pend_slices == 3 ? h->pend_part + 2 * h->pend_m * h->pend_c : nullptr, total4,
                     h->pend_c / 4);
  h->pend_bias = nullptr;
  DFOT_CHECK_HIP(hipGetLastError());
  return DFOT_OK;
}

static int run_tr_block(dfot_uvit_s* h, const TrW& w, int lvl, int batch, hipStream_t s) {
  const int c = w.c, rr = h->r[lvl], n = h->T * rr * rr, d = c / h->heads;
  const int m = batch * n;
  bf16* xb = h->XB[lvl];
  int rc = 0;
  if (h->pend_bias && (h->pend_lvl != lvl || h->pend_m != m || h->pend_c != c) && (rc = flush_pending(h, s))) return rc;
  if (!h->xin_bf[lvl]) {
    if ((rc = launch_f32_to_bf16(h->xin[lvl], xb, (long)m * c, s))) return rc;
    h->xin_bf[lvl] = true;
  }
  RmsPending pend{xb, h->pend_bias, h->pend_part, h->pend_part + (long)m * c, h->pend_slices == 3 ? h->pend_part + 2L * m * c : nullptr};
  if ((rc = launch_rms_film_bf16(xb, w.nw, w.fcache, h->sv + w.sv_off, h->have_mask ? h->cond_mask : nullptr, h->s1, m, c, rr * rr, h->T,
                                 h->cfg.eps, s, h->pend_bias ? &pend : nullptr)))
    return rc;
  h->pend_bias = nullptr;
  GemmArgs p;
  p.A = h->s1; p.lda = c; p.W = w.w_fused; p.M = m; p.N = 7 * c; p.K = c; p.bias = w.b_fused;
  p.out2 = h->cat + c; p.ldo2 = 5 * c; p.split = 3 * c;
  p.q = h->q; p.k = h->k; p.v = h->v; p.qw = w.qw; p.kw = w.kw; p.rope_cs = h->rope_cs[lvl]; p.heads = h->heads; p.d = d;
  p.ntok = n; p.qscale = 1.4426950408889634f / sqrtf((float)d); p.eps = h->cfg.eps;
  if ((rc = launch_gemm(A_DENSE, E_QKV, h->gemm_variant, p, s))) return rc;
  const bool timed = h->time_attn && lvl == 2 && h->ev_used < h->ev_start.size();
  if (timed) DFOT_CHECK_HIP(hipEventRecord(h->ev_start[h->ev_used], s));
  int av = h->attn_variant;
  if (av == 2 && d == 64 && n % 256 == 0) av = (attention_v5_applies(n, d, w.score_bound) && !h->attn_force_safe) ? 14 : 5;
  if ((rc = launch_attention(h->q, h->k, h->v, h->cat, 5 * c, batch, h->heads, n, d, av, s, &h->attn_scratch))) return rc;
  if (timed) DFOT_CHECK_HIP(hipEventRecord(h->ev_stop[h->ev_used++], s));
  GemmArgs o;
  o.A = h->cat; o.lda = 5 * c; o.W = w.w_out; o.M = m; o.N = c; o.K = 5 * c; o.bias = w.b_out; o.ldo = c;
  if (h->gemm_variant == GEMM_AUTO && h->out_part && (size_t)2 * m * c <= h->out_part_elems && m % 256 == 0 && c % 144 == 0 &&
      (long)(m / 256) * (c / 144) * 2 <= 256 && (5 * c / 64) >= 8) {
    GemmArgs p2 = o;
    p2.bias = nullptr; p2.out_f32 = h->out_part; p2.ksplit = 2; p2.slice_stride = (long)m * c;
    if ((rc = launch_gemm(A_DENSE, E_F32, GEMM_DMA3_256x144, p2, s))) return rc;
    h->pend_bias = w.b_out;
    h->pend_lvl = lvl; h->pend_m = m; h->pend_c = c; h->pend_slices = 2;
    swap_out_part(h);
    return DFOT_OK;
  }
  if (h->gemm_variant == GEMM_AUTO && c % 144 == 0 && m % 256 == 0 && (long)(m / 256) * ((c + 191) / 192) < 256 &&
      (long)(m / 256) * (c / 144) >= 200 && (long)(m / 256) * (c / 144) <= 256) {
    o.out_bf16 = xb;
    o.resid_bf = xb;
    return launch_gemm(A_DENSE, E_BF16, GEMM_DMA3_256x144, o, s);
  }
  o.out_f32 = h->X[lvl];
  if ((rc = launch_gemm(A_DENSE, E_F32, h->gemm_variant, o, s))) return rc;
  hipLaunchKernelGGL(add_f32_into_bf16_kernel, dim3(cdiv((long)m * c / 4, 256)), dim3(256), 0, s, xb, h->X[lvl], (long)m * c / 4);
  DFOT_CHECK_HIP(hipGetLastError());
  return DFOT_OK;
}


__global__ void slab_reduce_kernel(float* __restrict__ out, const float* __restrict__ bias, const float* __restrict__ slabs, int nslab, long stride4,
                                   long total4, int cq, const uint8_t* __restrict__ live, unsigned img4) {
  typedef __attribute__((ext_vector_type(4))) float f4;
  const long i = (long)blockIdx.x * blockDim.x + threadIdx.x;
  if (i >= total4) return;
  if (live && !live[(unsigned)i / img4]) return;
  f4 v = reinterpret_cast<const f4*>(bias)[i % cq];
  for (int sl = 0; sl < nslab; ++sl) v += reinterpret_cast<const f4*>(slabs)[sl * stride4 + i];
  reinterpret_cast<f4*>(out)[i] = v;
}

static int conv_between_levels(dfot_uvit_s* h, GemmArgs g, hipStream_t s) {
  const long px = (long)g.H * g.Wd;
  if (h->gemm_variant == GEMM_AUTO && h->out_part && !g.gn_part && g.M % 256 == 0 && px % 256 == 0 && (g.N % 144 == 0 || g.N == 256) &&
      (long)g.M * g.N < (1L << 31)) {
    const int bn = g.N % 144 == 0 ? 144 : 256;
    const int variant = bn == 144 ? GEMM_DMA3_256x144 : GEMM_DMA_256x256;
    const int tiles = (g.M / 256) * (g.N / bn);
    int ks = 1;
    while (tiles * ks * 2 <= 256 && g.K / 64 / (ks * 2) >= 16) ks *= 2;
    if (tiles * ks >= 192 && tiles * ks <= 256) {
      if (ks == 1) return launch_gemm(A_CONV3, E_F32, variant, g, s);
      if ((size_t)ks * g.M * g.N <= h->out_part_elems) {
        GemmArgs p = g;
        float* out = g.out_f32;
        const float* bias = g.bias;
        p.bias = nullptr; p.resid = nullptr; p.out_f32 = h->out_part; p.ksplit = ks; p.slice_stride = (long)g.M * g.N;
        int rc = launch_gemm(A_CONV3, E_F32, variant, p, s);
        if (rc) return rc;
        const long total4 = (long)g.M * g.N / 4;
        hipLaunchKernelGGL(slab_reduce_kernel, dim3(cdiv(total4, 256)), dim3(256), 0, s, out, bias, h->out_part, ks, total4, total4, g.N / 4, g.live,
                           (unsigned)(px * g.N / 4));
        DFOT_CHECK_HIP(hipGetLastError());
        return DFOT_OK;
      }
    }
  }
  return launch_gemm(A_CONV3, E_F32, h->gemm_variant, g, s);
}

static int run_down(dfot_uvit_s* h, int l, int bt, hipStream_t s, const uint8_t* live = nullptr) {
  const int rr = h->r[l], cin = h->ch[l], cout = h->ch[l + 1];
  int rc = 0;
// ... 248 lines not shown
    DFOT_CHECK_HIP(hipMemcpy(h->film_table, table.data(), table.size() * sizeof(FilmChunk), hipMemcpyHostToDevice));
    h->film_chunks = (int)table.size();
    if ((rc = dev_alloc(h, &h->cond_mask, (size_t)max_batch, true))) return rc;
    h->cond_batch = 0;
  }
  if ((rc = dev_alloc(h, &h->cat, mc * 5, true))) return rc;
  if ((rc = dev_alloc(h, &h->q, mc, true))) return rc;
  if ((rc = dev_alloc(h, &h->k, mc, true))) return rc;
  if ((rc = dev_alloc(h, &h->v, mc, true))) return rc;
  {
    const size_t e2 = bt * pix[2] * h->ch[2], e3 = bt * pix[3] * h->ch[3];
    h->out_part_elems = 3 * (e2 > e3 ? e2 : e3);
    if ((rc = dev_alloc(h, &h->out_part, h->out_part_elems, true))) return rc;
  }
  {
    size_t need = 16;
    for (int b = 1; b <= max_batch; ++b)
      for (int l = 2; l < 4; ++l) need = std::max(need, attention_scratch_bytes(b, h->heads, h->T * h->r[l] * h->r[l], h->ch[l] / h->heads));
    if ((rc = dev_alloc(h, &h->attn_scratch.p, need / sizeof(float), true))) return rc;
    h->attn_scratch.bytes = need;
  }
  h->max_batch = max_batch;
  return DFOT_OK;
}

size_t dfot_uvit_workspace_bytes(dfot_uvit_t h) { return h ? h->ws_bytes : 0; }

int dfot_uvit_attn_timing(dfot_uvit_t h, double* total_ms, int64_t* launches) {
  DFOT_REQUIRE(h && total_ms && launches, DFOT_ERR_ARG, "attn_timing: null argument");
  double tot = 0.0;
  for (size_t i = 0; i < h->ev_used; ++i) {
    DFOT_CHECK_HIP(hipEventSynchronize(h->ev_stop[i]));
    float ms = 0.f;
    DFOT_CHECK_HIP(hipEventElapsedTime(&ms, h->ev_start[i], h->ev_stop[i]));
    tot += ms;
  }
  *total_ms = tot;
  *launches = (int64_t)h->ev_used;
  h->ev_used = 0;
  return DFOT_OK;
}

int dfot_uvit_set_option(dfot_uvit_t h, const char* key, int value) {
  DFOT_REQUIRE(h && key, DFOT_ERR_ARG, "set_option: null argument");
  if (!strcmp(key, "gemm_variant")) h->gemm_variant = value;
  else if (!strcmp(key, "attn_variant")) h->attn_variant = value;
  else if (!strcmp(key, "attn_force_safe")) h->attn_force_safe = value != 0;
  else if (!strcmp(key, "time_attn")) {
    h->time_attn = value > 0;
    h->ev_used = 0;
    while ((int)h->ev_start.size() < value) {
      hipEvent_t a, b;
      DFOT_CHECK_HIP(hipEventCreate(&a));
      DFOT_CHECK_HIP(hipEventCreate(&b));
      h->ev_start.push_back(a);
      h->ev_stop.push_back(b);
    }
  }
  else {
    set_error("set_option: unknown key '%s'", key);
    return DFOT_ERR_ARG;
  }
  return DFOT_OK;
}

int dfot_uvit_query(dfot_uvit_t h, const char* key, double* value) {
  DFOT_REQUIRE(h && key && value, DFOT_ERR_ARG, "query: null argument");
  DFOT_REQUIRE(h->finalized, DFOT_ERR_STATE, "query: weights not finalized");
  float bound = 0.f;
  for (const TrW& w : h->down_tr) bound = fmaxf(bound, w.score_bound);
  for (const TrW& w : h->up_tr) bound = fmaxf(bound, w.score_bound);
  if (!strcmp(key, "score_bound_l2")) *value = bound;
  else if (!strcmp(key, "attn_kernel_l2")) *value = (bound < 64.0f && !h->attn_force_safe) ? 14 : 5;
  else if (!strcmp(key, "cond_builds")) *value = (double)h->cond_builds;
  else {
    set_error("query: unknown key '%s'", key);
    return DFOT_ERR_ARG;
  }
  return DFOT_OK;
}

int dfot_uvit_set_conditions(dfot_uvit_t h, const float* external_cond, const uint8_t* external_cond_mask, int batch,
                             void* stream) {
  DFOT_REQUIRE(h, DFOT_ERR_ARG, "set_conditions: null handle");
  DFOT_REQUIRE(!h->posefree, DFOT_ERR_STATE, "set_conditions: a pose-free handle (dfot_uvit3d_create) has no pose caches; call dfot_uvit3d_forward");
  DFOT_REQUIRE(external_cond != nullptr, DFOT_ERR_ARG, "External condition (camera pose) is required for U-ViT3DPose model.");
  DFOT_REQUIRE(h->finalized, DFOT_ERR_STATE, "set_conditions: weights not finalized");
  DFOT_REQUIRE(batch > 0 && batch <= h->max_batch, DFOT_ERR_STATE, "set_conditions: batch %d exceeds reserved %d", batch, h->max_batch);
  hipStream_t s = (hipStream_t)stream;
  const dfot_uvit_config& c = h->cfg;
  const int bt = batch * h->T, e = h->E;
  int rc = 0;
  h->cond_batch = 0;
  ++h->cond_builds;
  if ((rc = launch_cond_repack(external_cond, h->acond, bt, c.resolution, c.cond_dim, h->kpose, s))) return rc;
  {
    GemmArgs g;
    g.A = h->acond; g.lda = h->kpose; g.W = h->pose_w; g.M = bt * h->r[0] * h->r[0]; g.N = e; g.K = h->kpose;
    g.bias = h->pose_b; g.out_bf16 = h->emb[0]; g.ldo = e;
    if ((rc = launch_gemm(A_DENSE, E_BF16, h->gemm_variant, g, s))) return rc;
  }
  if ((rc = launch_emb_pyramid(h->emb[0], h->emb[1], h->emb[2], h->emb[3], bt, h->r[0], e, s))) return rc;
  auto fill = [&](bf16* fcache, const bf16* wf, int cc, int lvl) -> int {
    GemmArgs g;
    g.A = h->emb[lvl]; g.lda = e; g.W = wf; g.M = bt * h->r[lvl] * h->r[lvl]; g.N = 2 * cc; g.K = e;
    g.out_bf16 = fcache; g.ldo = 2 * cc;
    return launch_gemm(A_DENSE, E_BF16, h->gemm_variant, g, s);
  };
  for (int l = 0; l < 2; ++l) {
    for (ResW& w : h->down_res[l]) if ((rc = fill(w.fcache, w.w_film, w.c, l))) return rc;
    for (ResW& w : h->up_res[l]) if ((rc = fill(w.fcache, w.w_film, w.c, l))) return rc;
  }
  for (TrW& w : h->down_tr) if ((rc = fill(w.fcache, w.w_film, w.c, 2))) return rc;
  for (TrW& w : h->up_tr) if ((rc = fill(w.fcache, w.w_film, w.c, 2))) return rc;
  for (TrW& w : h->mid_tr) if ((rc = fill(w.fcache, w.w_film, w.c, 3))) return rc;
  h->have_mask = external_cond_mask != nullptr;
  if (h->have_mask) DFOT_CHECK_HIP(hipMemcpyAsync(h->cond_mask, external_cond_mask, batch, hipMemcpyDeviceToDevice, s));
  h->cond_batch = batch;
  return DFOT_OK;
}

int dfot_uvit_forward_cached(dfot_uvit_t h, const float* x, const float* noise_levels, float* out, int batch, void* stream) {
  return dfot_uvit_forward_cached_live(h, x, noise_levels, out, batch, nullptr, stream);
}

int dfot_uvit_forward_cached_live(dfot_uvit_t h, const float* x, const float* noise_levels, float* out, int batch, const uint8_t* live_frames,
                                  void* stream) {
  return dfot_uvit_forward_cached_masks(h, x, noise_levels, out, batch, live_frames, nullptr, stream);
}

int dfot_uvit_forward_cached_masks(dfot_uvit_t h, const float* x, const float* noise_levels, float* out, int batch, const uint8_t* live_frames,
                                   const uint8_t* fresh_frames, void* stream) {
  DFOT_REQUIRE(h && x && noise_levels && out, DFOT_ERR_ARG, "forward: null argument");
  DFOT_REQUIRE(!fresh_frames || h->last_batch == batch, DFOT_ERR_STATE,
               "forward: frozen frames need the previous forward of this handle to have run the same batch (%d, now %d)", h->last_batch, batch);
  DFOT_REQUIRE(!fresh_frames || live_frames, DFOT_ERR_ARG, "forward: frozen frames must also be dead frames (live_frames is null)");
  DFOT_REQUIRE(!h->posefree, DFOT_ERR_STATE, "forward_cached: a pose-free handle (dfot_uvit3d_create) runs through dfot_uvit3d_forward");
  DFOT_REQUIRE(h->finalized, DFOT_ERR_STATE, "forward: weights not finalized");
  DFOT_REQUIRE(batch > 0 && batch == h->cond_batch, DFOT_ERR_STATE,
               "forward_cached: batch %d does not match the cached conditions (%d)", batch, h->cond_batch);
  hipStream_t s = (hipStream_t)stream;
  const dfot_uvit_config& c = h->cfg;
  const int bt = batch * h->T, e = h->E;
  int rc = 0;
  if ((rc = launch_noise_emb(noise_levels, h->ne_freqs, h->ne_phases, h->ne_w1, h->ne_b1, h->ne_w2, h->ne_b2, h->nhid,
                             h->nemb, bt, c.noise_dim, e, s)))
    return rc;
  return forward_from_emb(h, x, out, batch, live_frames, fresh_frames, s);
}

}

static int forward_from_emb(dfot_uvit_s* h, const float* x, float* out, int batch, const uint8_t* live_frames, const uint8_t* fresh_frames,
                            hipStream_t s) {
  const dfot_uvit_config& c = h->cfg;
  const int bt = batch * h->T, e = h->E;
  int rc = 0;
  if ((rc = launch_film_vec(h->film_table, h->film_chunks, h->nemb, h->sv, bt, e, s))) return rc;
  if ((rc = launch_embed_input_bf16(x, h->ein_w, h->ein_b, h->XB[0], bt, c.resolution, c.in_channels, h->ch[0], s))) return rc;
  h->gn1_nblk = 0;
  for (int l = 0; l < 4; ++l) h->xin[l] = h->X[l];
  h->xin_bf[0] = true;
  h->xin_bf[1] = h->xin_bf[2] = h->xin_bf[3] = false;

  if (fresh_frames && (h->gemm_variant != GEMM_AUTO || (h->r[2] * h->r[2]) % 512 != 0)) fresh_frames = nullptr;
  for (int l = 0; l < 2; ++l) {
    for (const ResW& w : h->down_res[l])
      if ((rc = run_res_block(h, w, l, bt, s, fresh_frames))) return rc;
    if ((rc = run_down(h, l, bt, s, fresh_frames))) return rc;
  }
  h->pend_bias = nullptr;
  for (const TrW& w : h->down_tr)
    if ((rc = run_tr_block(h, w, 2, batch, s))) return rc;
  if ((rc = flush_pending(h, s))) return rc;
  if ((rc = run_down(h, 2, bt, s))) return rc;
  for (const TrW& w : h->mid_tr)
    if ((rc = run_tr_block(h, w, 3, batch, s))) return rc;
  if ((rc = flush_pending(h, s))) return rc;
  if ((rc = run_up(h, 2, bt, s))) return rc;
  for (const TrW& w : h->up_tr)
    if ((rc = run_tr_block(h, w, 2, batch, s))) return rc;
  if ((rc = flush_pending(h, s))) return rc;
  for (int l = 1; l >= 0; --l) {
    if ((rc = run_up(h, l, bt, s, live_frames))) return rc;
    for (const ResW& w : h->up_res[l])
      if ((rc = run_res_block(h, w, l, bt, s, live_frames))) return rc;
  }
  h->last_batch = batch;
  return launch_project_output_bf16(h->XB[0], h->pout_w, h->pout_b, out, bt, c.resolution, h->ch[0], c.in_channels, s, live_frames);
}

extern "C" {

int dfot_uvit_forward(dfot_uvit_t h, const float* x, const float* noise_levels, const float* external_cond,
                      const uint8_t* external_cond_mask, float* out, int batch, void* stream) {
  DFOT_REQUIRE(h && x && noise_levels && out, DFOT_ERR_ARG, "forward: null argument");
  int rc = dfot_uvit_set_conditions(h, external_cond, external_cond_mask, batch, stream);
  if (rc) return rc;
  return dfot_uvit_forward_cached(h, x, noise_levels, out, batch, stream);
}

int dfot_uvit3d_forward_live(dfot_uvit_t h, const float* x, const float* noise_levels, const float* external_cond,
                             const uint8_t* external_cond_mask, float* out, int batch, const uint8_t* live_frames, void* stream) {
  DFOT_REQUIRE(h && x && noise_levels && out, DFOT_ERR_ARG, "uvit3d_forward: null argument");
  DFOT_REQUIRE(h->posefree, DFOT_ERR_STATE, "uvit3d_forward: the handle is a pose model (dfot_uvit_create); call dfot_uvit_forward");
  DFOT_REQUIRE(h->finalized, DFOT_ERR_STATE, "uvit3d_forward: weights not finalized");
  DFOT_REQUIRE(batch > 0 && batch <= h->max_batch, DFOT_ERR_STATE, "uvit3d_forward: batch %d exceeds reserved %d", batch, h->max_batch);
  DFOT_REQUIRE(!external_cond || h->act_dim > 0, DFOT_ERR_ARG,
               "uvit3d_forward: external_cond given, but the model was built with cond_dim 0 (no external_cond_embedding)");
  hipStream_t s = (hipStream_t)stream;
  const uint8_t* mask = (external_cond && h->act_dropout) ? external_cond_mask : nullptr;
  int rc = launch_uvit3d_emb(noise_levels, h->ne_freqs, h->ne_phases, h->ne_w1, h->ne_b1, h->ne_w2, h->ne_b2, external_cond, mask, h->ac_w1,
                             h->ac_b1, h->ac_w2, h->ac_b2, h->nemb, batch * h->T, h->cfg.noise_dim, h->act_dim, h->E, h->T, s);
  if (rc) return rc;
  h->have_mask = false;
  return forward_from_emb(h, x, out, batch, live_frames, nullptr, s);
}

int dfot_uvit3d_forward(dfot_uvit_t h, const float* x, const float* noise_levels, const float* external_cond,
                        const uint8_t* external_cond_mask, float* out, int batch, void* stream) {
  return dfot_uvit3d_forward_live(h, x, noise_levels, external_cond, external_cond_mask, out, batch, nullptr, stream);
}

int dfot_op_gn_film_silu(const void* h, const float* stats, const float* gamma, const float* beta, const void* fcache, const float* sv,
                         const uint8_t* cond_mask, void* out, int bt, int pixels, int c, int tokens, void* stream) {
  DFOT_REQUIRE(h && stats && gamma && beta && sv && out, DFOT_ERR_ARG, "op_gn_film_silu: null argument");
  DFOT_REQUIRE(bt > 0 && pixels > 0 && tokens > 0 && c > 0 && c % 32 == 0, DFOT_ERR_SHAPE,
               "op_gn_film_silu: bt %d, pixels %d, tokens %d must be positive and channels %d a multiple of 32", bt, pixels, tokens, c);
  return launch_gn_film_silu((const bf16*)h, stats, gamma, beta, (const bf16*)fcache, sv, cond_mask, (bf16*)out, bt, pixels, c, tokens,
                             (hipStream_t)stream);
}
int dfot_op_rms_film(const void* x, const float* w, const void* fcache, const float* sv, const uint8_t* cond_mask, void* out, int64_t m,
                     int c, int rows_per_bt, int tokens, float eps, void* stream) {
  DFOT_REQUIRE(x && w && sv && out, DFOT_ERR_ARG, "op_rms_film: null argument");
  DFOT_REQUIRE(m > 0 && rows_per_bt > 0 && tokens > 0 && c > 0 && c % 32 == 0 && m % rows_per_bt == 0, DFOT_ERR_SHAPE,
               "op_rms_film: rows %ld must be a positive multiple of rows_per_bt %d, channels %d a multiple of 32", (long)m, rows_per_bt, c);
  return launch_rms_film_bf16((const bf16*)x, w, (const bf16*)fcache, sv, cond_mask, (bf16*)out, (long)m, c, rows_per_bt, tokens, eps,
                              (hipStream_t)stream);
}

int dfot_uvit_read_tap(dfot_uvit_t h, const char* name, float* out, size_t capacity, void* stream) {
  DFOT_REQUIRE(h && name && out, DFOT_ERR_ARG, "read_tap: null argument");
  DFOT_REQUIRE(h->last_batch > 0, DFOT_ERR_STATE, "read_tap: no forward has run");
  hipStream_t s = (hipStream_t)stream;
  const int bt = h->last_batch * h->T;
  if (!strcmp(name, "nemb")) {
    const size_t need = (size_t)bt * h->E;
    DFOT_REQUIRE(capacity >= need, DFOT_ERR_SHAPE, "read_tap: need %zu floats, got %zu", need, capacity);
    return copy_f32(out, h->nemb, need, s);
  }
  DFOT_REQUIRE(!(h->posefree && !strcmp(name, "pose_emb0")), DFOT_ERR_NAME, "read_tap: a pose-free handle has no tap 'pose_emb0'");
  auto pixels = [&](int l) { return h->r[l] * h->r[l]; };
  struct Tap { const char* n; int lvl; int c; const float* f; const bf16* b; };
  const Tap taps[] = {
      {"pose_emb0", 0, h->E, nullptr, h->emb[0]}, {"down0", 1, h->ch[1], h->HSA[0], nullptr},
      {"down1", 2, h->ch[2], h->HSA[1], nullptr}, {"down2", 3, h->ch[3], h->HSA[2], nullptr},
      {"mid", 3, h->ch[3], nullptr, h->XB[3]}, {"up2", 2, h->ch[2], nullptr, h->XB[2]},
      {"up1", 1, h->ch[1], nullptr, h->XB[1]}, {"up0", 0, h->ch[0], nullptr, h->XB[0]},
  };
  for (const Tap& t : taps) {
    if (strcmp(t.n, name)) continue;
    const size_t need = (size_t)bt * pixels(t.lvl) * t.c;
    DFOT_REQUIRE(capacity >= need, DFOT_ERR_SHAPE, "read_tap: need %zu floats, got %zu", need, capacity);
    return t.f ? launch_nhwc_to_nchw(t.f, out, bt, pixels(t.lvl), t.c, s)
               : launch_bf16_nhwc_to_nchw(t.b, out, bt, pixels(t.lvl), t.c, s);
  }
  set_error("read_tap: unknown tap '%s'", name);
  return DFOT_ERR_NAME;
}

int dfot_ray_encode(const float* raw_poses, float* out, int batch, int tokens, int resolution, void* stream) {
  DFOT_REQUIRE(raw_poses && out && batch > 0 && tokens > 0 && resolution > 0, DFOT_ERR_ARG, "ray_encode: bad argument");
  return launch_ray_encode(raw_poses, out, batch, tokens, resolution, 0, (hipStream_t)stream);
}

int dfot_ray_encode_normalized(const float* poses, float* out, int batch, int tokens, int resolution, void* stream) {
  DFOT_REQUIRE(poses && out && batch > 0 && tokens > 0 && resolution > 0, DFOT_ERR_ARG, "ray_encode_normalized: bad argument");
  return launch_ray_encode(poses, out, batch, tokens, resolution, 1, (hipStream_t)stream);
}

int dfot_hg_prepare(const float* x, const float* noise, const float* qa, const float* qb, float* x_in, int batch, int nfe,
                    int tokens, int64_t frame_elems, void* stream) {
  DFOT_REQUIRE(x && qa && qb && x_in, DFOT_ERR_ARG, "hg_prepare: null argument");
  return launch_hg_prepare(x, noise, qa, qb, x_in, batch, nfe, tokens, (long)frame_elems, (hipStream_t)stream);
}

int dfot_ddim_compose(const float* x, const float* x_in, const float* v, const float* sa, const float* s1, const float* an,
                      const float* cn, const float* keep, const float* weight, const uint8_t* gen, float* x_next, int batch,
                      int nfe, int tokens, int64_t frame_elems, void* stream) {
  DFOT_REQUIRE(x && x_in && v && sa && s1 && an && cn && keep && weight && gen && x_next, DFOT_ERR_ARG, "ddim_compose: null argument");
  return launch_ddim_compose(x, x_in, v, sa, s1, an, cn, keep, weight, gen, x_next, batch, nfe, tokens, (long)frame_elems, false,
                             (hipStream_t)stream);
}
int dfot_ddim_compose_tokw(const float* x, const float* x_in, const float* v, const float* sa, const float* s1, const float* an,
                           const float* cn, const float* keep, const float* weight, const uint8_t* gen, float* x_next, int batch,
                           int nfe, int tokens, int64_t frame_elems, void* stream) {
  DFOT_REQUIRE(x && x_in && v && sa && s1 && an && cn && keep && weight && gen && x_next, DFOT_ERR_ARG, "ddim_compose_tokw: null argument");
  return launch_ddim_compose(x, x_in, v, sa, s1, an, cn, keep, weight, gen, x_next, batch, nfe, tokens, (long)frame_elems, true,
                             (hipStream_t)stream);
}

int dfot_ddim_noise(const float* noise, const float* sigma, const float* weight, const uint8_t* gen, float* x_next, int batch, int nfe,
                    int tokens, int64_t frame_elems, int weight_per_token, void* stream) {
  DFOT_REQUIRE(noise && sigma && weight && gen && x_next, DFOT_ERR_ARG, "ddim_noise: null argument");
  return launch_ddim_noise(noise, sigma, weight, gen, x_next, batch, nfe, tokens, (long)frame_elems, weight_per_token != 0, (hipStream_t)stream);
}

int dfot_vpred_loss(const float* x, const float* noise, const float* v, const float* alpha, const float* sigma,
                    const float* weight, float* x_pred, float* scratch, float* loss, int batch, int tokens, int64_t frame_elems,
                    void* stream) {
  DFOT_REQUIRE(x && noise && v && alpha && sigma && weight && scratch && loss, DFOT_ERR_ARG, "vpred_loss: null argument");
  return launch_vloss(x, noise, v, alpha, sigma, weight, x_pred, scratch, loss, batch, tokens, (long)frame_elems, false,
                      (hipStream_t)stream);
}
int dfot_vspace_loss(const float* x, const float* noise, const float* v, const float* alpha, const float* sigma,
                     const float* weight, float* x_pred, float* scratch, float* loss, int batch, int tokens, int64_t frame_elems,
                     void* stream) {
  DFOT_REQUIRE(x && noise && v && alpha && sigma && weight && scratch && loss, DFOT_ERR_ARG, "vspace_loss: null argument");
  return launch_vloss(x, noise, v, alpha, sigma, weight, x_pred, scratch, loss, batch, tokens, (long)frame_elems, true,
                      (hipStream_t)stream);
}
int64_t dfot_vpred_loss_scratch_floats(int batch, int tokens, int64_t frame_elems) {
  return (int64_t)batch * tokens * vloss_chunks((long)frame_elems);
}

static bf16* g_zero_page = nullptr;
static int zero_page(bf16** out) {
  if (!g_zero_page) {
    DFOT_CHECK_HIP(hipMalloc((void**)&g_zero_page, 512));
    DFOT_CHECK_HIP(hipMemset(g_zero_page, 0, 512));
  }
  *out = g_zero_page;
  return DFOT_OK;
}

int dfot_op_gemm(const void* a, int lda, const void* w, const float* bias, float* c, int m, int n, int k, int variant,
                 void* stream) {
  GemmArgs g;
  g.A = (const bf16*)a; g.lda = lda; g.W = (const bf16*)w; g.M = m; g.N = n; g.K = k; g.bias = bias; g.out_f32 = c; g.ldo = n;
  DFOT_REQUIRE(c, DFOT_ERR_ARG, "op_gemm: null output");
  return launch_gemm(A_DENSE, E_F32, variant, g, (hipStream_t)stream);
}

int dfot_op_conv3x3(const void* a, const void* w, const float* bias, float* y, int bt, int hh, int ww, int cin, int cout,
                    int variant, void* stream) {
  GemmArgs g;
  int rc = zero_page(const_cast<bf16**>(&g.zeros));
  if (rc) return rc;
// ... 47 lines not shown
```

diffusion-forcing-transformer_amd/sampler.py:

```python
from __future__ import annotations

from dataclasses import dataclass, field
from typing import Callable, Dict, List, Optional, Tuple

import numpy as np
import torch

from . import capi, parallel
from .diffusion import DiffusionConfig, Schedule, denoising_loss, masked_mean
from .guidance import HistoryGuidance


@dataclass
class SamplerConfig:
    x_shape: Tuple[int, int, int] = (3, 256, 256)
    max_tokens: int = 8
    diffusion: DiffusionConfig = field(default_factory=DiffusionConfig)
    scheduling_matrix: str = "full_sequence"
    is_full_sequence: bool = False
    prediction_guidance: Dict = field(default_factory=lambda: {"name": "conditional"})
    interpolation_guidance: Dict = field(default_factory=lambda: {"name": "conditional"})
    keyframe_density: Optional[float] = None
    sliding_context_len: Optional[int] = None
    interpolation_max_batch_size: Optional[int] = None
    refinement_sampling: Optional[Dict] = None
    camera_pose_normalize_by: str = "first"
    camera_pose_bound: Optional[float] = None
    external_cond_type: str = "action"
    external_cond_dim: int = 0
    external_cond_processing: Optional[str] = None
    attention_map_steps: Tuple[int, ...] = ()


NoiseFn = Callable[[str, tuple], torch.Tensor]


def device_noise_fn(generator: Optional[torch.Generator] = None, clip: float = 20.0) -> NoiseFn:
    def fn(tag: str, shape: tuple) -> torch.Tensor:
        return torch.randn(shape, device="cuda", generator=generator).clamp_(-clip, clip)
    return fn


class DFoTVideoPoseSampler:
    def __init__(self, cfg: SamplerConfig, backbone, noise_fn: Optional[NoiseFn] = None):
        self.cfg = cfg
        self.model = backbone
        self.schedule = Schedule(cfg.diffusion)
        self.noise_fn = noise_fn or device_noise_fn(clip=cfg.diffusion.clip_noise)
        self.timesteps = cfg.diffusion.timesteps
        self.sampling_timesteps = cfg.diffusion.sampling_timesteps
        self.max_tokens = cfg.max_tokens
        self.x_shape = tuple(cfg.x_shape)
        self.trace: List[dict] = []
        self.window_forwards = 0
        self.shard_windows = False
        self.branch_parallel = False
        self._branch_split_active = False
        self.device = "cuda"
        self.dry_run = False
        self.use_graph = True
        self.skip_frozen_frames = True
        self.skip_dead_frames = True
        self.graph_replays = 0
        self.graph_captures = 0
        self._graphs: Dict[tuple, dict] = {}
        self._graphs_generation = 0
        self.attention_maps: Dict[int, dict] = {}
        if cfg.diffusion.sampling_timesteps > cfg.diffusion.timesteps:
            raise ValueError("sampling_timesteps must be <= timesteps")

    @torch.no_grad()
    def _process_conditions(self, conditions: Optional[torch.Tensor], noise_levels=None) -> Optional[torch.Tensor]:
        if conditions is None:
            return None
        if conditions.shape[-1] != 16:
            raise ValueError(f"raw camera poses must have 16 values per frame, got {conditions.shape[-1]}")
        cfg = self.cfg
        if cfg.camera_pose_normalize_by not in ("first", "mean"):
            raise ValueError(f"Unknown camera pose normalization method: {cfg.camera_pose_normalize_by}")
        interp = None
        if noise_levels is not None and getattr(self, "_interpolate_masked_poses", False):
            interp = np.asarray(noise_levels.detach().cpu().numpy() if torch.is_tensor(noise_levels) else noise_levels) == self.timesteps - 1
        if cfg.camera_pose_normalize_by == "first" and cfg.camera_pose_bound is None and interp is None:
            return torch.ops.dfot.ray_encoding(conditions, int(self.x_shape[-1]))
        from . import pose
        world = pose.normalize_poses(conditions.detach().float().cpu().numpy(), cfg.camera_pose_normalize_by, cfg.camera_pose_bound, interp)
        return torch.ops.dfot.ray_encoding(torch.from_numpy(world), int(self.x_shape[-1]), True)

    def _select_conditions(self, conditions: Optional[torch.Tensor], index) -> Optional[torch.Tensor]:
        return None if conditions is None else conditions[:, index]

    def _padded_conditions(self, conditions: Optional[torch.Tensor], index) -> Optional[torch.Tensor]:
        return None if conditions is None else self._pad_to_max_tokens(conditions[:, index])

    def _window_conditions(self, conditions: Optional[torch.Tensor]) -> Optional[torch.Tensor]:
        return self._process_conditions(conditions)

    def _check_conditions(self, conditions: Optional[torch.Tensor], length: int) -> None:
        pass

    _static_graph_cond = False

    @torch.no_grad()
    def denoising_loss(self, xs: torch.Tensor, conditions: Optional[torch.Tensor], t: torch.Tensor,
                       noise: Optional[torch.Tensor] = None, masks: Optional[torch.Tensor] = None):
        if noise is None:
            noise = self.noise_fn("train", tuple(xs.shape))
        _, per_token, x_pred, _ = denoising_loss(self.cfg.diffusion, lambda x_t, lv: self.model(x_t, lv, self._process_conditions(conditions), None),
                                                 xs, t, noise, want_x_pred=True)
        loss, per_token = masked_mean(per_token, masks)
        return x_pred, loss, per_token

    @torch.no_grad()
    def discrete_denoising_loss(self, xs: torch.Tensor, k: torch.Tensor, noise: Optional[torch.Tensor] = None,
                                masks: Optional[torch.Tensor] = None, loss_weighting: Optional[Dict] = None):
        if self.cfg.diffusion.is_continuous:
            raise ValueError("discrete_denoising_loss needs DiffusionConfig(is_continuous=False)")
        if noise is None:
            noise = self.noise_fn("train", tuple(xs.shape))
        _, per_token, x_pred, _ = denoising_loss(self.schedule, lambda x_k, lv: self.model(x_k, lv, None, None), xs, k, noise,
                                                 loss_weighting=loss_weighting, want_x_pred=True)
        loss, per_token = masked_mean(per_token, masks)
        return x_pred, loss, per_token

    def _normalize_x(self, xs: torch.Tensor, mean, std) -> torch.Tensor:
        m = torch.as_tensor(mean, dtype=xs.dtype, device=xs.device).view(-1, 1, 1)
        s = torch.as_tensor(std, dtype=xs.dtype, device=xs.device).view(-1, 1, 1)
        return (xs - m) / s

    def _unnormalize_x(self, xs: torch.Tensor, mean, std) -> torch.Tensor:
        m = torch.as_tensor(mean, dtype=xs.dtype, device=xs.device).view(-1, 1, 1)
        s = torch.as_tensor(std, dtype=xs.dtype, device=xs.device).view(-1, 1, 1)
        return xs * s + m

    def _pad_to_max_tokens(self, y: Optional[torch.Tensor]) -> Optional[torch.Tensor]:
        if y is None or y.shape[1] >= self.max_tokens:
            return y
        tail = y[:, -1:].expand(-1, self.max_tokens - y.shape[1], *y.shape[2:])
        return torch.cat([y, tail], dim=1)

    @torch.no_grad()
    def _sample_sequence(self, batch_size: int, length: Optional[int] = None, context: Optional[torch.Tensor] = None,
                         context_mask: Optional[torch.Tensor] = None, conditions: Optional[torch.Tensor] = None,
                         history_guidance: Optional[HistoryGuidance] = None, _refine: Optional[Tuple[int, int]] = None,
                         **_) -> Tuple[torch.Tensor, None]:
# ... 130 lines not shown
        if self.dry_run:
            for p_ in plans:
                if p_["nfe"] in split_nfe:
                    hb = parallel.world_info()[1] % p_["nfe"]
                    got = parallel.exchange_branches(torch.full((batch_size, 1), float(hb)), p_["nfe"])
                    if not torch.equal(got.view(batch_size, p_["nfe"]), torch.arange(p_["nfe"], dtype=got.dtype).repeat(batch_size, 1)):
                        raise RuntimeError("branch exchange returned the branches out of (sample, branch) order")
                    self.branch_exchanges = getattr(self, "branch_exchanges", 0) + 1
                if p_.get("renoise"):
                    self.noise_fn("renoise", (batch_size, horizon, *x_shape))
                    continue
                draw_noise(p_)
                if strict or p_["sigma"] is not None:
                    self.noise_fn("ddim", (p_["bm"], horizon, *x_shape))
                    if _refine is not None:
                        self.noise_fn("refine_context", (batch_size, horizon, *x_shape))
            self.window_forwards += sum(p_["bm"] for p_ in plans if not p_.get("renoise"))
            return (xs[:, :-padding] if padding > 0 else xs), None
        flat_dev = torch.from_numpy(np.concatenate([p_["tables"].ravel() for p_ in plans])).cuda()
        gens_dev = torch.from_numpy(np.stack([p_["gen"] for p_ in plans])).cuda()
        off = 0
        cmask_cache: Dict[bytes, torch.Tensor] = {}
        weight_cache: Dict[bytes, torch.Tensor] = {}
        lives_by_nfe: Dict[int, torch.Tensor] = {}
        for i, p_ in enumerate(plans):
            n = p_["tables"].size
            p_["tables_dev"] = flat_dev[off:off + n].view(8, p_["bm"], horizon)
            off += n
            p_["gen_dev"] = gens_dev[i]
            if p_.get("renoise"):
                continue
            if p_["nfe"] not in lives_by_nfe:
                lives_by_nfe[p_["nfe"]] = gens_dev if p_["nfe"] == 1 else gens_dev.repeat_interleave(p_["nfe"], dim=1)
            p_["live_dev"] = lives_by_nfe[p_["nfe"]][i]
            wsrc = p_["plan"].weights if p_["plan"].tok_weights is None else p_["plan"].tok_weights
            wkey = wsrc.tobytes()
            if wkey not in weight_cache:
                weight_cache[wkey] = torch.from_numpy(np.ascontiguousarray(wsrc, dtype=np.float32)).cuda()
            p_["weights_dev"] = weight_cache[wkey]
            p_["tokw"] = p_["plan"].tok_weights is not None
            p_["sigma_dev"] = None if p_["sigma"] is None else torch.from_numpy(p_["sigma"]).cuda()
            p_["cmask_dev"] = None
            if p_["cmask"] is not None:
                ckey = p_["cmask"].tobytes()
                if ckey not in cmask_cache:
                    cmask_cache[ckey] = torch.from_numpy(p_["cmask"]).cuda()
                p_["cmask_dev"] = cmask_cache[ckey]

        cond_full = None if pose_interp else self._window_conditions(conditions)
        cond_rep, cond_nfe = None, 0
        if pose_interp:
            by_mask: Dict[bytes, torch.Tensor] = {}
            self._interpolate_masked_poses = True
            try:
                for p_ in plans:
                    if p_.get("renoise"):
                        continue
                    lv = p_["plan"].levels.reshape(p_["bm"], horizon)
                    key = (lv == self.timesteps - 1).tobytes() + bytes([p_["nfe"]])
                    if key not in by_mask:
                        by_mask[key] = self._process_conditions(conditions.repeat_interleave(p_["nfe"], dim=0), lv)
                    p_["cond"] = by_mask[key]
            finally:
                self._interpolate_masked_poses = False
        fresh_dev = torch.from_numpy(np.concatenate([a.ravel() for a in self._fresh_flags(plans, batch_size, horizon)])).cuda()
        foff = 0
        for p_ in plans:
            p_["fresh_dev"] = fresh_dev[foff:foff + p_["bm"] * horizon].view(p_["bm"], horizon)
            foff += p_["bm"] * horizon
        xs = xs.contiguous()
        s = capi.stream_ptr
        branch_cache: Dict[tuple, tuple] = {}

        skip_dead = self.skip_dead_frames and hasattr(self.model, "live_frames")
        skip_frozen = skip_dead and self.skip_frozen_frames and hasattr(self.model, "fresh_frames")

        map_steps = set(int(i) for i in (getattr(cfg, "attention_map_steps", None) or ()))
        collect_at: Optional[int] = None
        if map_steps and not self.dry_run:
            if not hasattr(self.model, "capture_attention"):
                raise NotImplementedError(f"attention_map_steps: {type(self.model).__name__} has no attention-map capture (DiT3D backbones only)")
            self.attention_maps = {}

        def step(p_, xs, noise, tables, gen_dev, xs_next=None, live_dev=None, fresh_dev=None):
            nonlocal cond_rep, cond_nfe
            nfe, bm = p_["nfe"], p_["bm"]
            x_in = torch.empty(bm, horizon, *x_shape, device="cuda", dtype=torch.float32)
            capi.check(capi.lib.dfot_hg_prepare(capi.ptr(xs), capi.ptr(noise), capi.ptr(tables[0]), capi.ptr(tables[1]),
                                                capi.ptr(x_in), batch_size, nfe, horizon, f, s()))
            if cond_full is not None and cond_nfe != nfe:
                cond_rep = cond_full if nfe == 1 else cond_full.repeat_interleave(nfe, dim=0)
                cond_nfe = nfe
            if "cond" in p_:
                cond_rep = p_["cond"]
            lvl = tables[7] if cfg.diffusion.is_continuous else tables[7].to(torch.int32)
            world, rank = parallel.world_info()
            if nfe in split_nfe:
                hb = rank % nfe
                key = (id(cond_rep), id(p_["cmask_dev"]), hb)
                if key not in branch_cache:
                    c_h = None if cond_rep is None else cond_rep.view(batch_size, nfe, *cond_rep.shape[1:])[:, hb].contiguous()
                    m_h = None if p_["cmask_dev"] is None else p_["cmask_dev"].view(batch_size, nfe)[:, hb].contiguous()
                    branch_cache[key] = (c_h, m_h, cond_rep, p_["cmask_dev"])
                c_h, m_h = branch_cache[key][:2]
                x_h = x_in.view(batch_size, nfe, horizon, *x_shape)[:, hb].contiguous()
                l_h = lvl.view(batch_size, nfe, horizon)[:, hb].contiguous()
                if skip_dead:
                    self.model.live_frames = gen_dev
                try:
                    v = parallel.exchange_branches(self.model(x_h, l_h, c_h, m_h), nfe)
                    self.branch_exchanges = getattr(self, "branch_exchanges", 0) + 1
                finally:
                    if skip_dead:
                        self.model.live_frames = None
            elif rg > 0:
                v = self._reconstruction_guided_v(x_in, lvl, cond_rep, p_["cmask_dev"], tables, gen_dev, rg_ctx, rg, nfe)
            else:
                if skip_dead:
                    self.model.live_frames = live_dev if live_dev is not None else p_["live_dev"]
                if skip_frozen:
                    self.model.fresh_frames = fresh_dev if fresh_dev is not None else p_["fresh_dev"]
                try:
                    v = self.model(x_in, lvl, cond_rep, p_["cmask_dev"])
                finally:
                    if skip_dead:
                        self.model.live_frames = None
                    if skip_frozen:
                        self.model.fresh_frames = None
            if collect_at is not None:
                self.attention_maps[collect_at] = {"noise_levels": lvl.clone(), **self.model.attention_maps()}
            step_noise = None
            if strict or p_["sigma"] is not None:
                step_noise = self.noise_fn("ddim", (bm, horizon, *x_shape))
            if xs_next is None:
                xs_next = torch.empty_like(xs)
            compose = capi.lib.dfot_ddim_compose_tokw if p_["tokw"] else capi.lib.dfot_ddim_compose
            capi.check(compose(capi.ptr(xs), capi.ptr(x_in), capi.ptr(v), capi.ptr(tables[2]),
                                                  capi.ptr(tables[3]), capi.ptr(tables[4]), capi.ptr(tables[5]),
                                                  capi.ptr(tables[6]), capi.ptr(p_["weights_dev"]), capi.ptr(gen_dev),
                                                  capi.ptr(xs_next), batch_size, nfe, horizon, f, s()))
            if p_["sigma"] is not None:
                nz = step_noise.to(device="cuda", dtype=torch.float32).clamp(-cfg.diffusion.clip_noise, cfg.diffusion.clip_noise).contiguous()
                capi.check(capi.lib.dfot_ddim_noise(capi.ptr(nz), capi.ptr(p_["sigma_dev"]), capi.ptr(p_["weights_dev"]), capi.ptr(gen_dev),
                                                    capi.ptr(xs_next), batch_size, nfe, horizon, f, int(p_["tokw"]), s()))
            return xs_next

        def renoise(p_, xs):
            noise = self.noise_fn("renoise", (batch_size, horizon, *x_shape)).to(device="cuda", dtype=torch.float32)
            noise = noise.clamp(-cfg.diffusion.clip_noise, cfg.diffusion.clip_noise).contiguous()
            out = torch.empty_like(xs)
            capi.check(capi.lib.dfot_hg_prepare(capi.ptr(xs), capi.ptr(noise), capi.ptr(p_["tables_dev"][0]), capi.ptr(p_["tables_dev"][1]),
                                                capi.ptr(out), batch_size, 1, horizon, f, s()))
            return out

        if _refine is not None:
            for p_ in plans:
                if p_.get("renoise"):
                    xs = renoise(p_, xs)
                    continue
                xs = step(p_, xs, draw_noise(p_), p_["tables_dev"], p_["gen_dev"])
                if strict:
                    self.noise_fn("refine_context", (batch_size, horizon, *x_shape))
            self.window_forwards += sum(p_["bm"] for p_ in plans if not p_.get("renoise"))
            return (xs[:, :-padding] if padding > 0 else xs), None
        uniform = all(p_["bm"] == plans[0]["bm"] and p_["cmask_dev"] is plans[0]["cmask_dev"]
                      and p_["weights_dev"] is plans[0]["weights_dev"] and p_.get("cond") is plans[0].get("cond") for p_ in plans)
        hook = getattr(self, "step_hook", None)
        collecting = bool(map_steps) and not self.dry_run
        if (self.use_graph and uniform and not strict and len(plans) > 2 and all(p_["sigma"] is None for p_ in plans) and not self._branch_split_active
                and rg == 0 and hook is None and not collecting):
            if self._static_graph_cond and cond_full is not None:
                nfe0 = plans[0]["nfe"]
                plans[0]["cond_src"] = cond_full if nfe0 == 1 else cond_full.repeat_interleave(nfe0, dim=0)
            xs = self._run_steps_graph(plans, xs, draw_noise, step, flat_dev, gens_dev, horizon)
        else:
            own_capture = collecting and not self.model.capturing_attention
            if own_capture:
                self.model.capture_attention()
            try:
                for i, p_ in enumerate(plans):
                    collect_at = i if collecting and i in map_steps else None
                    xs = step(p_, xs, draw_noise(p_), p_["tables_dev"], p_["gen_dev"])
                    if hook is not None:
                        hook(i, xs)
            finally:
                collect_at = None
                if own_capture:
                    self.model.capture_attention(False)
        self.window_forwards += sum(p_["bm"] for p_ in plans)
        if padding > 0:
            xs = xs[:, :-padding]
        return xs, None

    @torch.no_grad()
    def _sample_sequence_refine(self, batch_size: int, goback_length: int, n_goback: int, length: Optional[int] = None,
                                context: Optional[torch.Tensor] = None, context_mask: Optional[torch.Tensor] = None,
                                conditions: Optional[torch.Tensor] = None, history_guidance: Optional[HistoryGuidance] = None,
                                **_) -> Tuple[torch.Tensor, None]:
        return self._sample_sequence(batch_size, length=length, context=context, context_mask=context_mask, conditions=conditions,
                                     history_guidance=history_guidance, _refine=(int(goback_length), int(n_goback)))

    def _window_sampler(self):
        return self._sample_sequence

    def _reconstruction_guided_v(self, x_in, lvl, cond, cmask, tables, gen_dev, ctx, rg: float, nfe: int):
        if nfe != 1:
            raise ValueError("reconstruction guidance needs one-branch history guidance (the reference's loss compares the "
                             "(B * NFE, ...) prediction with the (B, ...) context)")
        if self.cfg.diffusion.objective != "pred_v":
            raise ValueError("reconstruction guidance is implemented for the v objective")
        nd = x_in.ndim
        ext = lambda a: a.reshape(*a.shape, *([1] * (nd - a.ndim)))
        sa, s1 = ext(tables[2]), ext(tables[3])
        with torch.enable_grad():
            x = x_in.detach().requires_grad_(True)
            v = self.model(x, lvl, cond, cmask)
            pred_x0 = sa * x - s1 * v
            cm = ext((gen_dev == 0).to(torch.float32))
            loss = torch.sum((pred_x0 - ctx) ** 2 * sa * cm / cm.sum(dim=1, keepdim=True).clamp(min=1))
            grad = torch.nan_to_num(-torch.autograd.grad(-rg * 0.5 * loss, x)[0], nan=0.0)
        an, cn = ext(tables[4]), ext(tables[5])
        scale = torch.where(sa > 0, s1 / sa.clamp(min=1e-30), torch.where(an > 0, -cn / an.clamp(min=1e-30), torch.zeros_like(sa)))
        return (v.detach() + scale * grad).contiguous()

    @staticmethod
    def _fresh_flags(plans, batch_size: int, horizon: int):
        out, prev = [], None
        for p_ in plans:
            fresh = np.ones((p_["bm"], horizon), np.uint8)
            if p_.get("renoise"):
                out.append(fresh)
                prev = None
                continue
            if (prev is not None and prev["bm"] == p_["bm"] and prev["nfe"] == p_["nfe"] and prev.get("cond") is p_.get("cond")
                    and ((prev["cmask"] is None and p_["cmask"] is None)
                         or (prev["cmask"] is not None and p_["cmask"] is not None and np.array_equal(prev["cmask"], p_["cmask"])))):
                a, b = prev["tables"], p_["tables"]
                same_in = (a[0] == 1) & (a[1] == 0) & (b[0] == 1) & (b[1] == 0) & (a[7] == b[7])
                untouched = np.repeat(prev["gen"].reshape(batch_size, horizon) == 0, p_["nfe"], axis=0)
                fresh = np.where(same_in & untouched, 0, 1).astype(np.uint8)
            out.append(fresh)
            prev = p_
        return out

    def _run_steps_graph(self, plans, xs, draw_noise, step, flat_dev, gens_dev, horizon):
        p0 = plans[0]
        bm, n_steps, nfe = p0["bm"], len(plans), p0["nfe"]
        need_noise = any(p_["need_noise"] for p_ in plans)
        self.model.reserve(bm)
        if hasattr(self.model, "sync_weights"):
            self.model.sync_weights()
        gen = getattr(self.model, "reserve_generation", 0)
        if gen != self._graphs_generation:
            self._graphs.clear()
            self._graphs_generation = gen
        cond_src = p0.get("cond_src")
        key = (bm, n_steps, nfe, horizon, tuple(xs.shape), need_noise, None if p0["cmask"] is None else p0["cmask"].tobytes(),
               id(self.model), None if cond_src is None else (tuple(cond_src.shape), cond_src.dtype))
        ent = self._graphs.get(key)
        if ent is None:
            ent = dict(tables=torch.empty(n_steps, 8, bm, horizon, device="cuda", dtype=torch.float32),
                       gens=torch.empty_like(gens_dev), weights=torch.empty_like(p0["weights_dev"]),
                       lives=torch.empty(n_steps, bm, horizon, device="cuda", dtype=torch.uint8),
                       fresh=torch.empty(n_steps, bm, horizon, device="cuda", dtype=torch.uint8),
                       noise=torch.empty(n_steps, bm, *xs.shape[1:], device="cuda") if need_noise else None,
                       xs=torch.empty_like(xs), out=None, graph=None,
                       cond=None if cond_src is None else torch.empty_like(cond_src))
        ent["tables"].copy_(flat_dev.view(n_steps, 8, bm, horizon))
        ent["gens"].copy_(gens_dev)
        ent["lives"].copy_(gens_dev if nfe == 1 else gens_dev.repeat_interleave(nfe, dim=1))
        ent["fresh"].copy_(torch.stack([p_["fresh_dev"] for p_ in plans]))
        ent["weights"].copy_(p0["weights_dev"])
        if need_noise:
            for i, p_ in enumerate(plans):
                if p_["need_noise"]:
                    ent["noise"][i].copy_(draw_noise(p_))
                else:
                    ent["noise"][i].zero_()
        p_static = dict(p0, weights_dev=ent["weights"])
        if cond_src is not None:
            ent["cond"].copy_(cond_src)
            p_static["cond"] = ent["cond"]
        ent["xs"].copy_(step(p_static, xs, None if not need_noise else ent["noise"][0], ent["tables"][0], ent["gens"][0], live_dev=ent["lives"][0],
                            fresh_dev=ent["fresh"][0]))
        if ent["graph"] is None:
            torch.cuda.synchronize()
            graph = torch.cuda.CUDAGraph()
            with torch.cuda.graph(graph, capture_error_mode="thread_local"):
                x = ent["xs"]
                for i in range(1, n_steps):
                    x = step(p_static, x, ent["noise"][i] if need_noise else None, ent["tables"][i], ent["gens"][i], live_dev=ent["lives"][i],
                             fresh_dev=ent["fresh"][i])
                ent["out"] = x
            ent["graph"] = graph
            if len(self._graphs) >= 4:
                self._graphs.pop(next(iter(self._graphs)))
            self._graphs[key] = ent
            self.graph_captures += 1
        ent["graph"].replay()
        self.graph_replays += n_steps - 1
        return ent["out"].clone()

    @torch.no_grad()
    def _predict_sequence(self, context: torch.Tensor, length: Optional[int] = None,
                          conditions: Optional[torch.Tensor] = None, history_guidance: Optional[HistoryGuidance] = None,
                          sliding_context_len: Optional[int] = None, **_) -> Tuple[torch.Tensor, None]:
        mt = self.max_tokens
        if length is None:
            length = mt
        if sliding_context_len is None:
            if mt < length:
                raise ValueError("when length > max_tokens, sliding_context_len must be specified.")
            sliding_context_len = mt - 1
        if sliding_context_len == -1:
            sliding_context_len = mt - 1
        batch_size, gt_len = context.shape[:2]
        if sliding_context_len < gt_len:
            raise ValueError("sliding_context_len is expected to be >= length of initial context,"
                             f"got {sliding_context_len}. If you are trying to use max context, "
                             "consider specifying sliding_context_len=-1.")
        xs = context.to(device=self.device, dtype=torch.float32)
        cur = gt_len
        n_window = 0
        while cur < length:
            c = min(sliding_context_len, cur)
            h = min(length - cur, mt - c)
            window = torch.cat([xs[:, -c:], xs.new_zeros(batch_size, h, *self.x_shape)], 1)
            generated = cur - max(cur - c, gt_len)
            cmask = torch.ones(batch_size, c, dtype=torch.long)
            if generated > 0:
                cmask[:, -generated:] = 2
            cmask = torch.cat([cmask, torch.zeros(batch_size, h, dtype=torch.long)], 1)
            cond = self._select_conditions(conditions, slice(cur - c, cur - c + mt))
            if hasattr(self.noise_fn, "set_windows"):
                self.noise_fn.set_windows([n_window])
            n_window += 1
            new, _ = self._window_sampler()(batch_size, length=c + h, context=window, context_mask=cmask,
                                           conditions=cond, history_guidance=history_guidance)
            xs = torch.cat([xs, new[:, -h:]], 1)
            cur = xs.shape[1]
        return xs, None

    def _interpolation_plan(self, known: np.ndarray) -> List[List[np.ndarray]]:
        mt = self.max_tokens
        known = known.copy()
        plan: List[List[np.ndarray]] = []
        while not known.all():
            keys = np.where(known)[0]
            stage: List[np.ndarray] = []
            chunk: Optional[np.ndarray] = None
            for left, right in zip(keys[:-1], keys[1:]):
                left, right = int(left), int(right)
                if chunk is not None:
                    if len(chunk) + right - left <= mt:
                        chunk = np.concatenate([chunk, np.arange(left + 1, right + 1)])
                        continue
                    stage.append(chunk)
                    chunk = None
                if right - left == 1:
                    continue
                if right - left >= mt - 1:
                    stage.append(torch.linspace(left, right, mt).round().long().numpy())
                else:
                    chunk = np.arange(left, right + 1)
            if chunk is not None:
# ... 155 lines not shown
```

include/dfot_hip.h:

```cpp
#ifndef DFOT_HIP_H_
#define DFOT_HIP_H_

#include <stddef.h>
#include <stdint.h>

#ifdef __cplusplus
extern "C" {
#endif

enum {
  DFOT_OK = 0,
  DFOT_ERR_ARG = 1,
  DFOT_ERR_SHAPE = 2,
  DFOT_ERR_HIP = 3,
  DFOT_ERR_STATE = 4,
  DFOT_ERR_NAME = 5
};

typedef struct dfot_uvit_s* dfot_uvit_t;

typedef struct {
  int32_t channels[4];
  int32_t emb_channels;
  int32_t num_updown_blocks[3];
  int32_t num_mid_blocks;
  int32_t num_heads;
  int32_t in_channels;
  int32_t resolution;
  int32_t max_tokens;
  int32_t cond_dim;
  int32_t noise_dim;
  float rope_theta;
  float eps;
} dfot_uvit_config;

const char* dfot_last_error(void);
int dfot_version(void);

int dfot_uvit_create(const dfot_uvit_config* cfg, dfot_uvit_t* out);
int dfot_uvit_destroy(dfot_uvit_t h);
int dfot_uvit_num_params(dfot_uvit_t h);
const char* dfot_uvit_param_name(dfot_uvit_t h, int index);
int dfot_uvit_param_shape(dfot_uvit_t h, int index, int64_t shape[4], int* ndim);
int dfot_uvit_load_weight(dfot_uvit_t h, const char* name, const float* data, const int64_t* shape, int ndim,
                          void* stream);
int dfot_uvit_finalize(dfot_uvit_t h, void* stream);
int dfot_uvit_reserve(dfot_uvit_t h, int max_batch);
size_t dfot_uvit_workspace_bytes(dfot_uvit_t h);
int dfot_uvit_set_option(dfot_uvit_t h, const char* key, int value);
int dfot_uvit_query(dfot_uvit_t h, const char* key, double* value);
int dfot_uvit_attn_timing(dfot_uvit_t h, double* total_ms, int64_t* launches);

int dfot_uvit_forward(dfot_uvit_t h, const float* x, const float* noise_levels, const float* external_cond,
                      const uint8_t* external_cond_mask, float* out, int batch, void* stream);
int dfot_uvit_set_conditions(dfot_uvit_t h, const float* external_cond, const uint8_t* external_cond_mask, int batch,
                             void* stream);
int dfot_uvit_forward_cached(dfot_uvit_t h, const float* x, const float* noise_levels, float* out, int batch,
                             void* stream);
int dfot_uvit_forward_cached_live(dfot_uvit_t h, const float* x, const float* noise_levels, float* out, int batch,
                                  const uint8_t* live_frames, void* stream);
int dfot_uvit_forward_cached_masks(dfot_uvit_t h, const float* x, const float* noise_levels, float* out, int batch,
                                   const uint8_t* live_frames, const uint8_t* fresh_frames, void* stream);
int dfot_uvit_read_tap(dfot_uvit_t h, const char* name, float* out, size_t capacity_floats, void* stream);

typedef struct {
  int32_t channels[4];
  int32_t emb_channels;
  int32_t num_updown_blocks[3];
  int32_t num_mid_blocks;
  int32_t num_heads;
  int32_t in_channels;
  int32_t resolution;
  int32_t max_tokens;
  int32_t cond_dim;
  int32_t noise_dim;
  float rope_theta;
  float eps;
  int32_t cond_dropout;
} dfot_uvit3d_config;
int dfot_uvit3d_create(const dfot_uvit3d_config* cfg, dfot_uvit_t* out);
int64_t dfot_uvit3d_config_bytes(void);
int dfot_uvit3d_forward(dfot_uvit_t h, const float* x, const float* noise_levels, const float* external_cond,
                        const uint8_t* external_cond_mask, float* out, int batch, void* stream);
int dfot_uvit3d_forward_live(dfot_uvit_t h, const float* x, const float* noise_levels, const float* external_cond,
                             const uint8_t* external_cond_mask, float* out, int batch, const uint8_t* live_frames, void* stream);
int dfot_op_gn_film_silu(const void* h, const float* stats, const float* gamma, const float* beta, const void* fcache, const float* sv,
                         const uint8_t* cond_mask, void* out, int bt, int pixels, int c, int tokens, void* stream);
int dfot_op_rms_film(const void* x, const float* w, const void* fcache, const float* sv, const uint8_t* cond_mask, void* out, int64_t m,
                     int c, int rows_per_bt, int tokens, float eps, void* stream);

typedef struct dfot_dit_s* dfot_dit_t;

typedef struct {
  int32_t hidden_size;
  int32_t depth;
  int32_t num_heads;
  int32_t patch_size;
  int32_t in_channels;
  int32_t height;
  int32_t width;
  int32_t max_tokens;
  int32_t mlp_hidden;
  int32_t noise_dim;
  int32_t timesteps;
  float rope_theta;
  float eps;
  int32_t variant;
  int32_t embed_col_dim;
  int32_t num_col_heads;
  int32_t num_row_heads;
  int32_t temporal_mlp_hidden;
  int32_t use_bias;
  int32_t cond_type;
  int32_t cond_dim;
  int32_t num_classes;
  int32_t cond_dropout;
  int32_t use_temporal_rope;
} dfot_dit_config;
enum { DFOT_COND_NONE = 0, DFOT_COND_ACTION = 1, DFOT_COND_LABEL = 2 };

typedef struct {
  dfot_dit_config base;
  int32_t fourier_noise;
} dfot_dit_config_f;

int dfot_dit_create(const dfot_dit_config* cfg, dfot_dit_t* out);
int dfot_dit_create_f(const dfot_dit_config_f* cfg, dfot_dit_t* out);
int dfot_dit_destroy(dfot_dit_t h);
int dfot_dit_num_params(dfot_dit_t h);
const char* dfot_dit_param_name(dfot_dit_t h, int index);
int dfot_dit_param_shape(dfot_dit_t h, int index, int64_t shape[4], int* ndim);
int dfot_dit_load_weight(dfot_dit_t h, const char* name, const float* data, const int64_t* shape, int ndim, void* stream);
int dfot_dit_finalize(dfot_dit_t h, void* stream);
int dfot_dit_reserve(dfot_dit_t h, int max_batch);
size_t dfot_dit_workspace_bytes(dfot_dit_t h);
int dfot_dit_set_option(dfot_dit_t h, const char* key, int value);
int dfot_dit_attn_timing(dfot_dit_t h, double* total_ms, int64_t* launches);
int dfot_dit_forward(dfot_dit_t h, const float* x, const int32_t* noise_levels, float* out, int batch, int tokens,
                     void* stream);
int dfot_dit_forward_cond(dfot_dit_t h, const float* x, const int32_t* noise_levels, const float* cond, const int32_t* labels,
                          const uint8_t* cond_mask, float* out, int batch, int tokens, void* stream);
int dfot_dit_forward_f(dfot_dit_t h, const float* x, const float* noise_levels, const float* cond, const int32_t* labels,
                       const uint8_t* cond_mask, float* out, int batch, int tokens, void* stream);
int dfot_dit_read_tap(dfot_dit_t h, const char* name, float* out, size_t capacity_floats, void* stream);
int dfot_op_dit_final_layer(const float* x, const float* table, const int32_t* levels, int64_t ldt, int64_t off, const float* w, const float* b,
                            float* out, int hidden, int rows_per_frame, int rows, float eps, int max_level, int c, int h, int width, int patch,
                            int form, void* stream);
int dfot_op_dit_final_layer_chunked(const float* x, const float* table, const int32_t* levels, int64_t ldt, int64_t off, const float* w,
                                    const float* b, float* out, int hidden, int rows_per_frame, int rows, float eps, int max_level, int c, int h,
                                    int width, int patch, int chunk, void* stream);

enum { DFOT_ATTN_MAP_OFF = -1, DFOT_ATTN_MAP_FRAME = 0, DFOT_ATTN_MAP_FULL = 1 };
int dfot_dit_capture_attention(dfot_dit_t h, const int32_t* blocks, int count, int form, size_t max_bytes);
int dfot_dit_attention_map_shape(dfot_dit_t h, int slot, int64_t shape[5], int* ndim);
int dfot_dit_read_attention_map(dfot_dit_t h, int slot, float* out, size_t capacity_floats, void* stream);

typedef struct dfot_dit_train_s* dfot_dit_train_t;
int dfot_dit_train_create(const dfot_dit_config* cfg, dfot_dit_train_t* out);
int dfot_dit_train_create_f(const dfot_dit_config_f* cfg, dfot_dit_train_t* out);
int dfot_facmat_train_create(const dfot_dit_config_f* cfg, dfot_dit_train_t* out);
int dfot_facdit_train_create(const dfot_dit_config_f* cfg, dfot_dit_train_t* out);
int dfot_dit_train_destroy(dfot_dit_train_t h);
int dfot_dit_train_num_params(dfot_dit_train_t h);
const char* dfot_dit_train_param_name(dfot_dit_train_t h, int i);
int dfot_dit_train_param_shape(dfot_dit_train_t h, int i, int64_t shape[4], int* ndim);
int64_t dfot_dit_train_param_offset(dfot_dit_train_t h, int i);
int64_t dfot_dit_train_total_numel(dfot_dit_train_t h);
size_t dfot_dit_train_workspace_bytes(dfot_dit_train_t h);
int dfot_dit_train_attach(dfot_dit_train_t h, float* params, float* grads);
int dfot_dit_train_reserve(dfot_dit_train_t h, int max_batch);
int dfot_dit_train_sync_weights(dfot_dit_train_t h, void* stream);
int dfot_dit_train_forward(dfot_dit_train_t h, const float* x, const int32_t* noise_levels, float* out, int batch, int tokens, void* stream);
// ... 210 lines not shown
```

Baseline: 10.82.

## Share pose-condition cache across guidance branches instead of repeating per branch

When the sampler runs several guidance branches (nfe>1) in one batch, it now passes the unrepeated camera conditions together with a group factor, rather than repeat_interleaving them per branch. The condition-embedding build and the cached FiLM tensors are computed once per sample. The groupnorm-FiLM and RMS-FiLM kernels gain a grouped template that remaps each model row to its shared condition row. This reduces condition build work and fcache memory traffic, at the cost of extra index arithmetic and more template variants.

```diff
diff --git a/diffusion-forcing-transformer_amd/backbone.py b/diffusion-forcing-transformer_amd/backbone.py
--- a/diffusion-forcing-transformer_amd/backbone.py
+++ b/diffusion-forcing-transformer_amd/backbone.py
@@ -80,6 +80,7 @@
         self._trainer_sig = None
         self.live_frames = None
         self.fresh_frames = None
+        self.cond_group = 1
         self._fresh_key = None
         self._train_stamp = 0
         self._dropout_generator: Optional[torch.Generator] = None
@@ -256,12 +257,12 @@
             out.append(eng.dx_in.to(grad_out.dtype))
         return out
 
-    def _cond_content_equal(self, cond: torch.Tensor, mask: Optional[torch.Tensor]) -> bool:
+    def _cond_content_equal(self, cond: torch.Tensor, mask: Optional[torch.Tensor], group: int = 1) -> bool:
         if self._cond_key is None or self._cond_refs is None:
             return False
         kept, kept_mask = self._cond_refs
-        _, version, shape, synced, mask_key = self._cond_key
-        if synced != self._synced or self._cond_gen != self.reserve_generation:
+        _, version, shape, synced, mask_key, kept_group = self._cond_key
+        if synced != self._synced or self._cond_gen != self.reserve_generation or kept_group != group:
             return False
         if kept._version != version or (kept_mask is not None and kept_mask._version != mask_key[1]):
             return False
@@ -295,10 +296,15 @@
         b = x.shape[0]
         if tuple(x.shape[2:]) != self.x_shape:
             raise ValueError(f"x has frame shape {tuple(x.shape[2:])}, expected {self.x_shape}")
-        if tuple(external_cond.shape) != (b, self.temporal_length, self.external_cond_dim, *self.x_shape[1:]):
-            raise ValueError(f"external_cond has shape {tuple(external_cond.shape)}")
+        group = int(self.cond_group)
+        if group < 1 or b % group != 0:
+            raise ValueError(f"cond_group {group} does not divide the model batch {b}")
+        if tuple(external_cond.shape) != (b // group, self.temporal_length, self.external_cond_dim, *self.x_shape[1:]):
+            raise ValueError(f"external_cond has shape {tuple(external_cond.shape)}" + (f" (cond_group {group})" if group > 1 else ""))
         if external_cond_mask is not None:
             assert external_cond_mask.ndim == 1, "embedding mask should be of shape (B,)"
+            if group > 1 and external_cond_mask.shape[0] != b:
+                raise ValueError(f"external_cond_mask has {external_cond_mask.shape[0]} entries, expected one per model row ({b})")
         if tuple(noise_levels.shape) != (b, self.temporal_length):
             raise ValueError(f"noise_levels has shape {tuple(noise_levels.shape)}, expected {(b, self.temporal_length)}")
         dev = next(self.parameters()).device
@@ -310,17 +316,18 @@
         xf = x.detach().to(torch.float32).contiguous()
         kf = noise_levels.detach().to(torch.float32).contiguous()
         key = (external_cond.data_ptr(), external_cond._version, tuple(external_cond.shape), self._synced,
-               None if external_cond_mask is None else (external_cond_mask.data_ptr(), external_cond_mask._version))
+               None if external_cond_mask is None else (external_cond_mask.data_ptr(), external_cond_mask._version), group)
         if key == self._cond_key:
             self.cond_cache_stats["identity_hits"] += 1
         else:
-            if self._cond_content_equal(external_cond, external_cond_mask):
+            if self._cond_content_equal(external_cond, external_cond_mask, group):
                 self.cond_cache_stats["content_hits"] += 1
             else:
                 cf = external_cond.detach().to(torch.float32).contiguous()
                 mf = None if external_cond_mask is None else external_cond_mask.to(torch.uint8).contiguous()
-                capi.check(capi.lib.dfot_uvit_set_conditions(self._handle, capi.ptr(cf, torch.float32, "external_cond"),
-                                                             capi.ptr(mf, torch.uint8, "external_cond_mask"), b, capi.stream_ptr()))
+                capi.check(capi.lib.dfot_uvit_set_conditions_grouped(self._handle, capi.ptr(cf, torch.float32, "external_cond"),
+                                                                     capi.ptr(mf, torch.uint8, "external_cond_mask"), b, group,
+                                                                     capi.stream_ptr()))
                 self.cond_cache_stats["builds"] += 1
             self._cond_key = key
             self._cond_refs = (external_cond, external_cond_mask)
diff --git a/diffusion-forcing-transformer_amd/capi.py b/diffusion-forcing-transformer_amd/capi.py
--- a/diffusion-forcing-transformer_amd/capi.py
+++ b/diffusion-forcing-transformer_amd/capi.py
@@ -89,6 +89,7 @@
     "dfot_uvit_attn_timing": (_I, [_P, C.POINTER(C.c_double), C.POINTER(_L)]),
     "dfot_uvit_forward": (_I, [_P, _P, _P, _P, _P, _P, _I, _P]),
     "dfot_uvit_set_conditions": (_I, [_P, _P, _P, _I, _P]),
+    "dfot_uvit_set_conditions_grouped": (_I, [_P, _P, _P, _I, _I, _P]),
     "dfot_uvit_forward_cached": (_I, [_P, _P, _P, _P, _I, _P]),
     "dfot_uvit_forward_cached_live": (_I, [_P, _P, _P, _P, _I, _P, _P]),
     "dfot_uvit_forward_cached_masks": (_I, [_P, _P, _P, _P, _I, _P, _P, _P]),
@@ -99,6 +100,8 @@
     "dfot_uvit3d_forward_live": (_I, [_P, _P, _P, _P, _P, _P, _I, _P, _P]),
     "dfot_op_gn_film_silu": (_I, [_P, _P, _P, _P, _P, _P, _P, _P, _I, _I, _I, _I, _P]),
     "dfot_op_rms_film": (_I, [_P, _P, _P, _P, _P, _P, _L, _I, _I, _I, _F, _P]),
+    "dfot_op_gn_film_silu_grouped": (_I, [_P, _P, _P, _P, _P, _P, _P, _P, _P, _I, _I, _I, _I, _I, _P]),
+    "dfot_op_rms_film_grouped": (_I, [_P, _P, _P, _P, _P, _P, _L, _I, _I, _I, _F, _I, _P, _P, _P, _P]),
     "dfot_dit_create": (_I, [C.POINTER(DiTConfig), C.POINTER(_P)]),
     "dfot_dit_create_f": (_I, [C.POINTER(DiTConfigF), C.POINTER(_P)]),
     "dfot_dit_destroy": (_I, [_P]),
diff --git a/diffusion-forcing-transformer_amd/csrc/kernels.h b/diffusion-forcing-transformer_amd/csrc/kernels.h
--- a/diffusion-forcing-transformer_amd/csrc/kernels.h
+++ b/diffusion-forcing-transformer_amd/csrc/kernels.h
@@ -29,7 +29,7 @@
 int launch_film_vec(const FilmChunk* table, int chunks, const float* nemb, float* sv, int bt, int e, hipStream_t s);
 int launch_gn_film_silu(const bf16* h, const float* stats, const float* gamma, const float* beta, const bf16* fcache,
                         const float* sv, const uint8_t* cond_mask, bf16* out, int bt, int pixels, int c, int tokens,
-                        hipStream_t s, const uint8_t* live = nullptr);
+                        hipStream_t s, const uint8_t* live = nullptr, int group = 1);
 struct RmsPending {
   void* x;
   const float* bias;
@@ -38,9 +38,9 @@
   const float* s2;
 };
 int launch_rms_film(const float* x, const float* w, const bf16* fcache, const float* sv, const uint8_t* cond_mask, bf16* out,
-                    long m, int c, int rows_per_bt, int tokens, float eps, hipStream_t s, const RmsPending* pend = nullptr);
+                    long m, int c, int rows_per_bt, int tokens, float eps, hipStream_t s, const RmsPending* pend = nullptr, int group = 1);
 int launch_rms_film_bf16(const bf16* x, const float* w, const bf16* fcache, const float* sv, const uint8_t* cond_mask, bf16* out,
-                         long m, int c, int rows_per_bt, int tokens, float eps, hipStream_t s, const RmsPending* pend = nullptr);
+                         long m, int c, int rows_per_bt, int tokens, float eps, hipStream_t s, const RmsPending* pend = nullptr, int group = 1);
 
 int launch_pool2_bf16(const float* x, bf16* out, int bt, int h, int w, int c, hipStream_t s);
 int launch_pool2_bf16_bf16in(const bf16* x, bf16* out, int bt, int h, int w, int c, hipStream_t s);
diff --git a/diffusion-forcing-transformer_amd/csrc/kernels.hip b/diffusion-forcing-transformer_amd/csrc/kernels.hip
--- a/diffusion-forcing-transformer_amd/csrc/kernels.hip
+++ b/diffusion-forcing-transformer_amd/csrc/kernels.hip
@@ -744,18 +744,23 @@
   return DFOT_OK;
 }
 
-template <bool POSE>
+template <bool POSE, bool GRP>
 __global__ void gn_film_silu_kernel(const bf16* __restrict__ h, const float* __restrict__ stats,
                                     const float* __restrict__ gamma, const float* __restrict__ beta,
                                     const bf16* __restrict__ fcache, const float* __restrict__ sv,
                                     const uint8_t* __restrict__ cond_mask, bf16* __restrict__ out, long total8, int pixels,
-                                    int c, int tokens, const uint8_t* __restrict__ live) {
+                                    int c, int tokens, const uint8_t* __restrict__ live, int group) {
   const long idx = (long)blockIdx.x * blockDim.x + threadIdx.x;
   if (idx >= total8) return;
   const unsigned iu = (unsigned)idx, cq = (unsigned)(c / 8);
   const int c8 = (int)(iu % cq);
   const long pix = iu / cq;
+  long fpix = pix;
   const int bt = (int)((unsigned)pix / (unsigned)pixels);
+  if constexpr (GRP) {
+    const unsigned mrow = (unsigned)bt / (unsigned)tokens;
+    fpix = pix - (long)(mrow - mrow / (unsigned)group) * tokens * pixels;
+  }
   if (live && !live[bt]) return;
   const int cpg = c / 32;
   const int c0 = c8 * 8;
@@ -771,8 +776,8 @@
   if constexpr (POSE) {
     const bool use_pose = !(cond_mask && cond_mask[(unsigned)bt / (unsigned)tokens]);
     if (use_pose) {
-      const bf16x8 fs = *reinterpret_cast<const bf16x8*>(fcache + pix * 2 * c + col);
-      const bf16x8 fh = *reinterpret_cast<const bf16x8*>(fcache + pix * 2 * c + col + 32);
+      const bf16x8 fs = *reinterpret_cast<const bf16x8*>(fcache + fpix * 2 * c + col);
+      const bf16x8 fh = *reinterpret_cast<const bf16x8*>(fcache + fpix * 2 * c + col + 32);
 #pragma unroll
       for (int j = 0; j < 8; ++j) {
         sc[j] += bf2f(fs[j]);
@@ -791,15 +796,20 @@
   }
   *reinterpret_cast<bf16x8*>(out + pix * c + c0) = o;
 }
-template <int C, bool POSE>
+template <int C, bool POSE, bool GRP>
 __global__ __launch_bounds__(256) void gn_film_silu_rows_kernel(const bf16* __restrict__ h, const float* __restrict__ stats,
                                                                 const float* __restrict__ gamma, const float* __restrict__ beta,
                                                                 const bf16* __restrict__ fcache, const float* __restrict__ sv,
                                                                 const uint8_t* __restrict__ cond_mask, bf16* __restrict__ out, int pixels,
-                                                                int tokens, const uint8_t* __restrict__ live) {
+                                                                int tokens, const uint8_t* __restrict__ live, int group) {
   constexpr int TPP = C / 8, PPI = 256 / TPP;
   const int wg_per_bt = pixels / (PPI * GN_ROWS_IT);
-  const int bt = blockIdx.x / wg_per_bt;
+  int bt = blockIdx.x / wg_per_bt;
+  int fbt = bt;
+  if constexpr (GRP) {
+    const unsigned mrow = (unsigned)bt / (unsigned)tokens;
+    fbt = (int)(mrow / (unsigned)group * (unsigned)tokens + ((unsigned)bt - mrow * (unsigned)tokens));
+  }
   if (live && !live[bt]) return;
   const int c0 = (threadIdx.x % TPP) * 8;
   const int col = (c0 >> 5) * 64 + (c0 & 31);
@@ -819,12 +829,14 @@
   bool use_pose = false;
   if constexpr (POSE) use_pose = !(cond_mask && cond_mask[(unsigned)bt / (unsigned)tokens]);
   long pix = (long)bt * pixels + (long)(blockIdx.x % wg_per_bt) * (PPI * GN_ROWS_IT) + threadIdx.x / TPP;
+  long fpix = pix - (long)(bt - fbt) * pixels;
   if (POSE && use_pose) {
 #pragma unroll 4
-    for (int it = 0; it < GN_ROWS_IT; ++it, pix += PPI) {
+    for (int it = 0; it < GN_ROWS_IT; ++it, pix += PPI, fpix += PPI) {
+      const long fp = GRP ? fpix : pix;
       const bf16x8 hv = *reinterpret_cast<const bf16x8*>(h + pix * C + c0);
-      const bf16x8 fs = *reinterpret_cast<const bf16x8*>(fcache + pix * 2 * C + col);
-      const bf16x8 fh = *reinterpret_cast<const bf16x8*>(fcache + pix * 2 * C + col + 32);
+      const bf16x8 fs = *reinterpret_cast<const bf16x8*>(fcache + fp * 2 * C + col);
+      const bf16x8 fh = *reinterpret_cast<const bf16x8*>(fcache + fp * 2 * C + col + 32);
       bf16x8 o;
 #pragma unroll
       for (int j = 0; j < 8; ++j) {
@@ -845,42 +857,53 @@
   }
 }
 
-template <bool POSE>
+template <bool POSE, bool GRP>
 static int launch_gn_film_silu_t(const bf16* h, const float* stats, const float* gamma, const float* beta, const bf16* fcache,
                                  const float* sv, const uint8_t* cond_mask, bf16* out, int bt, int pixels, int c, int tokens,
-                                 hipStream_t s, const uint8_t* live) {
+                                 hipStream_t s, const uint8_t* live, int group) {
   if ((c == 128 || c == 256) && pixels % ((256 / (c / 8)) * GN_ROWS_IT) == 0) {
     const int grid = bt * (pixels / ((256 / (c / 8)) * GN_ROWS_IT));
     if (c == 128)
-      hipLaunchKernelGGL((gn_film_silu_rows_kernel<128, POSE>), dim3(grid), dim3(256), 0, s, h, stats, gamma, beta, fcache, sv, cond_mask, out, pixels, tokens, live);
+      hipLaunchKernelGGL((gn_film_silu_rows_kernel<128, POSE, GRP>), dim3(grid), dim3(256), 0, s, h, stats, gamma, beta, fcache, sv, cond_mask, out, pixels, tokens, live, group);
     else
-      hipLaunchKernelGGL((gn_film_silu_rows_kernel<256, POSE>), dim3(grid), dim3(256), 0, s, h, stats, gamma, beta, fcache, sv, cond_mask, out, pixels, tokens, live);
+      hipLaunchKernelGGL((gn_film_silu_rows_kernel<256, POSE, GRP>), dim3(grid), dim3(256), 0, s, h, stats, gamma, beta, fcache, sv, cond_mask, out, pixels, tokens, live, group);
     DFOT_CHECK_HIP(hipGetLastError());
     return DFOT_OK;
   }
   const long total8 = (long)bt * pixels * (c / 8);
   DFOT_REQUIRE(total8 < (1L << 31), DFOT_ERR_SHAPE, "groupnorm apply: %ld work items exceed the 32-bit index range", total8);
-  hipLaunchKernelGGL(gn_film_silu_kernel<POSE>, dim3(cdiv(total8, 256)), dim3(256), 0, s, h, stats, gamma, beta, fcache, sv,
-                     cond_mask, out, total8, pixels, c, tokens, live);
+  hipLaunchKernelGGL((gn_film_silu_kernel<POSE, GRP>), dim3(cdiv(total8, 256)), dim3(256), 0, s, h, stats, gamma, beta, fcache, sv,
+                     cond_mask, out, total8, pixels, c, tokens, live, group);
   DFOT_CHECK_HIP(hipGetLastError());
   return DFOT_OK;
 }
 int launch_gn_film_silu(const bf16* h, const float* stats, const float* gamma, const float* beta, const bf16* fcache,
                         const float* sv, const uint8_t* cond_mask, bf16* out, int bt, int pixels, int c, int tokens,
-                        hipStream_t s, const uint8_t* live) {
-  return fcache ? launch_gn_film_silu_t<true>(h, stats, gamma, beta, fcache, sv, cond_mask, out, bt, pixels, c, tokens, s, live)
-                : launch_gn_film_silu_t<false>(h, stats, gamma, beta, nullptr, sv, nullptr, out, bt, pixels, c, tokens, s, live);
-}
-
-template <int MAXCH, bool PEND, typename TS, bool POSE>
+                        hipStream_t s, const uint8_t* live, int group) {
+  DFOT_REQUIRE(group == 1 || (group > 1 && tokens > 0 && bt % (group * tokens) == 0), DFOT_ERR_SHAPE,
+               "groupnorm apply: %d frames are not whole groups of %d rows x %d tokens", bt, group, tokens);
+  if (fcache && group > 1)
+    return launch_gn_film_silu_t<true, true>(h, stats, gamma, beta, fcache, sv, cond_mask, out, bt, pixels, c, tokens, s, live, group);
+  return fcache ? launch_gn_film_silu_t<true, false>(h, stats, gamma, beta, fcache, sv, cond_mask, out, bt, pixels, c, tokens, s, live, 1)
+                : launch_gn_film_silu_t<false, false>(h, stats, gamma, beta, nullptr, sv, nullptr, out, bt, pixels, c, tokens, s, live, 1);
+}
+
+template <int MAXCH, bool PEND, typename TS, bool POSE, bool GRP>
 __global__ __launch_bounds__(256) void rms_film_kernel(const TS* x, const float* __restrict__ w,
                                                        const bf16* __restrict__ fcache, const float* __restrict__ sv,
                                                        const uint8_t* __restrict__ cond_mask, bf16* __restrict__ out,
                                                        long m, int c, int rows_per_bt, int tokens, float eps, TS* xw,
                                                        const float* __restrict__ pbias, const float* __restrict__ p0,
-                                                       const float* __restrict__ p1, const float* __restrict__ p2) {
+                                                       const float* __restrict__ p1, const float* __restrict__ p2, int group) {
   const long row = (long)blockIdx.x * 4 + (threadIdx.x >> 6);
   if (row >= m) return;
+  long frow = row;
+  if constexpr (GRP) {
+    const unsigned wv = __builtin_amdgcn_readfirstlane((unsigned)row);
+    const unsigned nper = (unsigned)(tokens * rows_per_bt);
+    const unsigned mrow = wv / nper;
+    frow = row - (long)(mrow - mrow / (unsigned)group) * nper;
+  }
   const int lane = threadIdx.x & 63;
   const int nch = c / 8;
   const TS* src = x + row * c;
@@ -930,8 +953,8 @@
         sh[j] = svp[32 + j];
       }
       if (POSE && use_pose) {
-        const bf16x8 fs = *reinterpret_cast<const bf16x8*>(fcache + row * 2 * c + col);
-        const bf16x8 fh = *reinterpret_cast<const bf16x8*>(fcache + row * 2 * c + col + 32);
+        const bf16x8 fs = *reinterpret_cast<const bf16x8*>(fcache + (GRP ? frow : row) * 2 * c + col);
+        const bf16x8 fh = *reinterpret_cast<const bf16x8*>(fcache + (GRP ? frow : row) * 2 * c + col + 32);
 #pragma unroll
         for (int j = 0; j < 8; ++j) {
           sc[j] += bf2f(fs[j]);
@@ -945,13 +968,13 @@
     }
   }
 }
-template <typename TS, bool POSE>
+template <typename TS, bool POSE, bool GRP>
 static int launch_rms_film_p(const TS* x, const float* w, const bf16* fcache, const float* sv, const uint8_t* cond_mask, bf16* out,
-                             long m, int c, int rows_per_bt, int tokens, float eps, hipStream_t s, const RmsPending* pend) {
+                             long m, int c, int rows_per_bt, int tokens, float eps, hipStream_t s, const RmsPending* pend, int group) {
   DFOT_REQUIRE(c % 8 == 0 && c <= 8 * 64 * 3, DFOT_ERR_SHAPE, "rms_film: channels %d unsupported", c);
 #define RMS_CALL(MC, P)                                                                                                             \
-  hipLaunchKernelGGL((rms_film_kernel<MC, P, TS, POSE>), dim3(cdiv(m, 4)), dim3(256), 0, s, x, w, fcache, sv, cond_mask, out, m, c, rows_per_bt, \
-                     tokens, eps, P ? (TS*)pend->x : nullptr, P ? pend->bias : nullptr, P ? pend->s0 : nullptr, P ? pend->s1 : nullptr, P ? pend->s2 : nullptr)
+  hipLaunchKernelGGL((rms_film_kernel<MC, P, TS, POSE, GRP>), dim3(cdiv(m, 4)), dim3(256), 0, s, x, w, fcache, sv, cond_mask, out, m, c, rows_per_bt, \
+                     tokens, eps, P ? (TS*)pend->x : nullptr, P ? pend->bias : nullptr, P ? pend->s0 : nullptr, P ? pend->s1 : nullptr, P ? pend->s2 : nullptr, group)
   if (pend) {
     DFOT_REQUIRE(pend->x && pend->bias && pend->s0 && pend->s1, DFOT_ERR_ARG, "rms_film: pending sum needs a target, a bias and two slices");
     if (c <= 8 * 64 * 2) RMS_CALL(2, true); else RMS_CALL(3, true);
@@ -964,17 +987,21 @@
 }
 template <typename TS>
 static int launch_rms_film_t(const TS* x, const float* w, const bf16* fcache, const float* sv, const uint8_t* cond_mask, bf16* out,
-                             long m, int c, int rows_per_bt, int tokens, float eps, hipStream_t s, const RmsPending* pend) {
-  return fcache ? launch_rms_film_p<TS, true>(x, w, fcache, sv, cond_mask, out, m, c, rows_per_bt, tokens, eps, s, pend)
-                : launch_rms_film_p<TS, false>(x, w, nullptr, sv, nullptr, out, m, c, rows_per_bt, tokens, eps, s, pend);
+                             long m, int c, int rows_per_bt, int tokens, float eps, hipStream_t s, const RmsPending* pend, int group) {
+  DFOT_REQUIRE(group == 1 || (group > 1 && tokens > 0 && rows_per_bt > 0 && m % ((long)group * tokens * rows_per_bt) == 0), DFOT_ERR_SHAPE,
+               "rms_film: %ld rows are not whole groups of %d rows x %d tokens x %d", m, group, tokens, rows_per_bt);
+  DFOT_REQUIRE(group == 1 || m < (1L << 31), DFOT_ERR_SHAPE, "rms_film: %ld rows exceed the 32-bit index range of the grouped form", m);
+  if (fcache && group > 1) return launch_rms_film_p<TS, true, true>(x, w, fcache, sv, cond_mask, out, m, c, rows_per_bt, tokens, eps, s, pend, group);
+  return fcache ? launch_rms_film_p<TS, true, false>(x, w, fcache, sv, cond_mask, out, m, c, rows_per_bt, tokens, eps, s, pend, 1)
+                : launch_rms_film_p<TS, false, false>(x, w, nullptr, sv, nullptr, out, m, c, rows_per_bt, tokens, eps, s, pend, 1);
 }
 int launch_rms_film(const float* x, const float* w, const bf16* fcache, const float* sv, const uint8_t* cond_mask, bf16* out,
-                    long m, int c, int rows_per_bt, int tokens, float eps, hipStream_t s, const RmsPending* pend) {
-  return launch_rms_film_t<float>(x, w, fcache, sv, cond_mask, out, m, c, rows_per_bt, tokens, eps, s, pend);
+                    long m, int c, int rows_per_bt, int tokens, float eps, hipStream_t s, const RmsPending* pend, int group) {
+  return launch_rms_film_t<float>(x, w, fcache, sv, cond_mask, out, m, c, rows_per_bt, tokens, eps, s, pend, group);
 }
 int launch_rms_film_bf16(const bf16* x, const float* w, const bf16* fcache, const float* sv, const uint8_t* cond_mask, bf16* out,
-                         long m, int c, int rows_per_bt, int tokens, float eps, hipStream_t s, const RmsPending* pend) {
-  return launch_rms_film_t<bf16>(x, w, fcache, sv, cond_mask, out, m, c, rows_per_bt, tokens, eps, s, pend);
+                         long m, int c, int rows_per_bt, int tokens, float eps, hipStream_t s, const RmsPending* pend, int group) {
+  return launch_rms_film_t<bf16>(x, w, fcache, sv, cond_mask, out, m, c, rows_per_bt, tokens, eps, s, pend, group);
 }
 
 template <typename TIN>
diff --git a/diffusion-forcing-transformer_amd/csrc/uvit.hip b/diffusion-forcing-transformer_amd/csrc/uvit.hip
--- a/diffusion-forcing-transformer_amd/csrc/uvit.hip
+++ b/diffusion-forcing-transformer_amd/csrc/uvit.hip
@@ -98,6 +98,7 @@
   uint8_t* cond_mask = nullptr;
   bool have_mask = false;
   int cond_batch = 0;
+  int cond_group = 1;
   int64_t cond_builds = 0;
   bf16 *acond = nullptr, *emb[4] = {nullptr, nullptr, nullptr, nullptr}, *s1 = nullptr, *hbf = nullptr,
        *cat = nullptr, *q = nullptr, *k = nullptr, *v = nullptr;
@@ -386,7 +387,7 @@
   if ((rc = launch_gemm(A_CONV3, E_BF16, h->gemm_variant, g, s))) return rc;
   if ((rc = launch_gn_finalize(h->gn_partial2, h->gn_stats, bt, slots, pix, c, h->cfg.eps, s))) return rc;
   if ((rc = launch_gn_film_silu(h->hbf, h->gn_stats, w.g2, w.be2, w.fcache, h->sv + w.sv_off,
-                                h->have_mask ? h->cond_mask : nullptr, h->s1, bt, pix, c, h->T, s, live)))
+                                h->have_mask ? h->cond_mask : nullptr, h->s1, bt, pix, c, h->T, s, live, w.fcache ? h->cond_group : 1)))
     return rc;
   GemmArgs o;
   o.A = h->s1; o.W = w.w2; o.M = m; o.N = c; o.K = 9 * c; o.H = rr; o.Wd = rr; o.Cin = c; o.zeros = h->zeros;
@@ -443,7 +444,7 @@
   }
   RmsPending pend{xb, h->pend_bias, h->pend_part, h->pend_part + (long)m * c, h->pend_slices == 3 ? h->pend_part + 2L * m * c : nullptr};
   if ((rc = launch_rms_film_bf16(xb, w.nw, w.fcache, h->sv + w.sv_off, h->have_mask ? h->cond_mask : nullptr, h->s1, m, c, rr * rr, h->T,
-                                 h->cfg.eps, s, h->pend_bias ? &pend : nullptr)))
+                                 h->cfg.eps, s, h->pend_bias ? &pend : nullptr, w.fcache ? h->cond_group : 1)))
     return rc;
   h->pend_bias = nullptr;
   GemmArgs p;
@@ -858,14 +859,20 @@
 
 int dfot_uvit_set_conditions(dfot_uvit_t h, const float* external_cond, const uint8_t* external_cond_mask, int batch,
                              void* stream) {
+  return dfot_uvit_set_conditions_grouped(h, external_cond, external_cond_mask, batch, 1, stream);
+}
+
+int dfot_uvit_set_conditions_grouped(dfot_uvit_t h, const float* external_cond, const uint8_t* external_cond_mask, int batch, int group,
+                                     void* stream) {
   DFOT_REQUIRE(h, DFOT_ERR_ARG, "set_conditions: null handle");
   DFOT_REQUIRE(!h->posefree, DFOT_ERR_STATE, "set_conditions: a pose-free handle (dfot_uvit3d_create) has no pose caches; call dfot_uvit3d_forward");
   DFOT_REQUIRE(external_cond != nullptr, DFOT_ERR_ARG, "External condition (camera pose) is required for U-ViT3DPose model.");
   DFOT_REQUIRE(h->finalized, DFOT_ERR_STATE, "set_conditions: weights not finalized");
   DFOT_REQUIRE(batch > 0 && batch <= h->max_batch, DFOT_ERR_STATE, "set_conditions: batch %d exceeds reserved %d", batch, h->max_batch);
+  DFOT_REQUIRE(group >= 1 && batch % group == 0, DFOT_ERR_SHAPE, "set_conditions: batch %d is not a whole number of groups of %d", batch, group);
   hipStream_t s = (hipStream_t)stream;
   const dfot_uvit_config& c = h->cfg;
-  const int bt = batch * h->T, e = h->E;
+  const int bt = (batch / group) * h->T, e = h->E;
   int rc = 0;
   h->cond_batch = 0;
   ++h->cond_builds;
@@ -893,6 +900,7 @@
   h->have_mask = external_cond_mask != nullptr;
   if (h->have_mask) DFOT_CHECK_HIP(hipMemcpyAsync(h->cond_mask, external_cond_mask, batch, hipMemcpyDeviceToDevice, s));
   h->cond_batch = batch;
+  h->cond_group = group;
   return DFOT_OK;
 }
 
@@ -1015,6 +1023,31 @@
                               (hipStream_t)stream);
 }
 
+int dfot_op_gn_film_silu_grouped(const void* h, const float* stats, const float* gamma, const float* beta, const void* fcache,
+                                 const float* sv, const uint8_t* cond_mask, const uint8_t* live, void* out, int bt, int pixels, int c,
+                                 int tokens, int group, void* stream) {
+  DFOT_REQUIRE(h && stats && gamma && beta && sv && out, DFOT_ERR_ARG, "op_gn_film_silu_grouped: null argument");
+  DFOT_REQUIRE(bt > 0 && pixels > 0 && tokens > 0 && c > 0 && c % 32 == 0, DFOT_ERR_SHAPE,
+               "op_gn_film_silu_grouped: bt %d, pixels %d, tokens %d must be positive and channels %d a multiple of 32", bt, pixels, tokens, c);
+  DFOT_REQUIRE(group >= 1 && bt % (group * tokens) == 0, DFOT_ERR_SHAPE,
+               "op_gn_film_silu_grouped: %d frames are not whole groups of %d rows x %d tokens", bt, group, tokens);
+  return launch_gn_film_silu((const bf16*)h, stats, gamma, beta, (const bf16*)fcache, sv, cond_mask, (bf16*)out, bt, pixels, c, tokens,
+                             (hipStream_t)stream, live, group);
+}
+int dfot_op_rms_film_grouped(void* x, const float* w, const void* fcache, const float* sv, const uint8_t* cond_mask, void* out, int64_t m,
+                             int c, int rows_per_bt, int tokens, float eps, int group, const float* pend_bias, const float* pend_s0,
+                             const float* pend_s1, void* stream) {
+  DFOT_REQUIRE(x && w && sv && out, DFOT_ERR_ARG, "op_rms_film_grouped: null argument");
+  DFOT_REQUIRE(m > 0 && rows_per_bt > 0 && tokens > 0 && c > 0 && c % 32 == 0 && m % rows_per_bt == 0, DFOT_ERR_SHAPE,
+               "op_rms_film_grouped: rows %ld must be a positive multiple of rows_per_bt %d, channels %d a multiple of 32", (long)m, rows_per_bt, c);
+  DFOT_REQUIRE(group >= 1 && m % ((int64_t)group * tokens * rows_per_bt) == 0, DFOT_ERR_SHAPE,
+               "op_rms_film_grouped: %ld rows are not whole groups of %d rows x %d tokens x %d", (long)m, group, tokens, rows_per_bt);
+  DFOT_REQUIRE(!pend_bias || (pend_s0 && pend_s1), DFOT_ERR_ARG, "op_rms_film_grouped: a pending bias needs its two slices");
+  RmsPending pend{x, pend_bias, pend_s0, pend_s1, nullptr};
+  return launch_rms_film_bf16((const bf16*)x, w, (const bf16*)fcache, sv, cond_mask, (bf16*)out, (long)m, c, rows_per_bt, tokens, eps,
+                              (hipStream_t)stream, pend_bias ? &pend : nullptr, group);
+}
+
 int dfot_uvit_read_tap(dfot_uvit_t h, const char* name, float* out, size_t capacity, void* stream) {
   DFOT_REQUIRE(h && name && out, DFOT_ERR_ARG, "read_tap: null argument");
   DFOT_REQUIRE(h->last_batch > 0, DFOT_ERR_STATE, "read_tap: no forward has run");
@@ -1036,10 +1069,11 @@
   };
   for (const Tap& t : taps) {
     if (strcmp(t.n, name)) continue;
-    const size_t need = (size_t)bt * pixels(t.lvl) * t.c;
+    const int tbt = t.b == h->emb[0] ? bt / h->cond_group : bt;
+    const size_t need = (size_t)tbt * pixels(t.lvl) * t.c;
     DFOT_REQUIRE(capacity >= need, DFOT_ERR_SHAPE, "read_tap: need %zu floats, got %zu", need, capacity);
-    return t.f ? launch_nhwc_to_nchw(t.f, out, bt, pixels(t.lvl), t.c, s)
-               : launch_bf16_nhwc_to_nchw(t.b, out, bt, pixels(t.lvl), t.c, s);
+    return t.f ? launch_nhwc_to_nchw(t.f, out, tbt, pixels(t.lvl), t.c, s)
+               : launch_bf16_nhwc_to_nchw(t.b, out, tbt, pixels(t.lvl), t.c, s);
   }
   set_error("read_tap: unknown tap '%s'", name);
   return DFOT_ERR_NAME;
diff --git a/diffusion-forcing-transformer_amd/sampler.py b/diffusion-forcing-transformer_amd/sampler.py
--- a/diffusion-forcing-transformer_amd/sampler.py
+++ b/diffusion-forcing-transformer_amd/sampler.py
@@ -61,6 +61,7 @@
         self.use_graph = True
         self.skip_frozen_frames = True
         self.skip_dead_frames = True
+        self.share_branch_conditions = True
         self.graph_replays = 0
         self.graph_captures = 0
         self._graphs: Dict[tuple, dict] = {}
@@ -357,17 +358,24 @@
                 raise NotImplementedError(f"attention_map_steps: {type(self.model).__name__} has no attention-map capture (DiT3D backbones only)")
             self.attention_maps = {}
 
+        def shares_conditions(nfe):
+            return (self.share_branch_conditions and nfe > 1 and nfe not in split_nfe and rg == 0 and hasattr(self.model, "cond_group"))
+
         def step(p_, xs, noise, tables, gen_dev, xs_next=None, live_dev=None, fresh_dev=None):
             nonlocal cond_rep, cond_nfe
             nfe, bm = p_["nfe"], p_["bm"]
             x_in = torch.empty(bm, horizon, *x_shape, device="cuda", dtype=torch.float32)
             capi.check(capi.lib.dfot_hg_prepare(capi.ptr(xs), capi.ptr(noise), capi.ptr(tables[0]), capi.ptr(tables[1]),
                                                 capi.ptr(x_in), batch_size, nfe, horizon, f, s()))
-            if cond_full is not None and cond_nfe != nfe:
+            cond_group = 1
+            if "cond" in p_:
+                cond_rep = p_["cond"]
+                cond_group = p_.get("cond_group", 1)
+            elif cond_full is not None and shares_conditions(nfe):
+                cond_rep, cond_nfe, cond_group = cond_full, 0, nfe
+            elif cond_full is not None and cond_nfe != nfe:
                 cond_rep = cond_full if nfe == 1 else cond_full.repeat_interleave(nfe, dim=0)
                 cond_nfe = nfe
-            if "cond" in p_:
-                cond_rep = p_["cond"]
             lvl = tables[7] if cfg.diffusion.is_continuous else tables[7].to(torch.int32)
             world, rank = parallel.world_info()
             if nfe in split_nfe:
@@ -395,9 +403,13 @@
                     self.model.live_frames = live_dev if live_dev is not None else p_["live_dev"]
                 if skip_frozen:
                     self.model.fresh_frames = fresh_dev if fresh_dev is not None else p_["fresh_dev"]
+                if cond_group > 1:
+                    self.model.cond_group = cond_group
                 try:
                     v = self.model(x_in, lvl, cond_rep, p_["cmask_dev"])
                 finally:
+                    if cond_group > 1:
+                        self.model.cond_group = 1
                     if skip_dead:
                         self.model.live_frames = None
                     if skip_frozen:
@@ -446,7 +458,10 @@
                 and rg == 0 and hook is None and not collecting):
             if self._static_graph_cond and cond_full is not None:
                 nfe0 = plans[0]["nfe"]
-                plans[0]["cond_src"] = cond_full if nfe0 == 1 else cond_full.repeat_interleave(nfe0, dim=0)
+                if shares_conditions(nfe0):
+                    plans[0]["cond_src"], plans[0]["cond_src_group"] = cond_full, nfe0
+                else:
+                    plans[0]["cond_src"] = cond_full if nfe0 == 1 else cond_full.repeat_interleave(nfe0, dim=0)
             xs = self._run_steps_graph(plans, xs, draw_noise, step, flat_dev, gens_dev, horizon)
         else:
             own_capture = collecting and not self.model.capturing_attention
@@ -556,6 +571,7 @@
         if cond_src is not None:
             ent["cond"].copy_(cond_src)
             p_static["cond"] = ent["cond"]
+            p_static["cond_group"] = p0.get("cond_src_group", 1)
         ent["xs"].copy_(step(p_static, xs, None if not need_noise else ent["noise"][0], ent["tables"][0], ent["gens"][0], live_dev=ent["lives"][0],
                             fresh_dev=ent["fresh"][0]))
         if ent["graph"] is None:
diff --git a/include/dfot_hip.h b/include/dfot_hip.h
--- a/include/dfot_hip.h
+++ b/include/dfot_hip.h
@@ -55,6 +55,8 @@
                       const uint8_t* external_cond_mask, float* out, int batch, void* stream);
 int dfot_uvit_set_conditions(dfot_uvit_t h, const float* external_cond, const uint8_t* external_cond_mask, int batch,
                              void* stream);
+int dfot_uvit_set_conditions_grouped(dfot_uvit_t h, const float* external_cond, const uint8_t* external_cond_mask, int batch, int group,
+                                     void* stream);
 int dfot_uvit_forward_cached(dfot_uvit_t h, const float* x, const float* noise_levels, float* out, int batch,
                              void* stream);
 int dfot_uvit_forward_cached_live(dfot_uvit_t h, const float* x, const float* noise_levels, float* out, int batch,
@@ -88,6 +90,12 @@
                          const uint8_t* cond_mask, void* out, int bt, int pixels, int c, int tokens, void* stream);
 int dfot_op_rms_film(const void* x, const float* w, const void* fcache, const float* sv, const uint8_t* cond_mask, void* out, int64_t m,
                      int c, int rows_per_bt, int tokens, float eps, void* stream);
+int dfot_op_gn_film_silu_grouped(const void* h, const float* stats, const float* gamma, const float* beta, const void* fcache,
+                                 const float* sv, const uint8_t* cond_mask, const uint8_t* live, void* out, int bt, int pixels, int c,
+                                 int tokens, int group, void* stream);
+int dfot_op_rms_film_grouped(void* x, const float* w, const void* fcache, const float* sv, const uint8_t* cond_mask, void* out, int64_t m,
+                             int c, int rows_per_bt, int tokens, float eps, int group, const float* pend_bias, const float* pend_s0,
+                             const float* pend_s1, void* stream);
 
 typedef struct dfot_dit_s* dfot_dit_t;
 
```

Result: no change. 10.84, median of 2 (+0.1%).
